# ningyu1991/InclusiveGAN

Measured on AMD Instinct MI355X. Metric: training img/sec (whole node), CelebA 128x128 StyleGAN2+IMLE, higher is better.
Workload: dtype f32-equivalent (3x3 convs: 2-piece fp16 split, operands to <= 1 ulp of fp32, scales per pixel / per channel: no per-tensor window; fp32 sums)

## Files before the change

### include/igan_hip.h

```cpp
#ifndef IGAN_HIP_H
#define IGAN_HIP_H

#include <stddef.h>
#include <stdint.h>

#ifdef __cplusplus
extern "C" {
#endif

#define IGAN_ABI_VERSION 10

typedef void* igan_stream_t;

enum igan_status {
    IGAN_OK = 0,
    IGAN_ERR_INVALID_ARGUMENT = 1,
    IGAN_ERR_HIP = 2,
    IGAN_ERR_UNSUPPORTED = 3
};

int igan_abi_version(void);
size_t igan_struct_size(int which);
const char* igan_last_error(void);

typedef struct igan_upfirdn2d_params {
    const float* x;
    const float* k;
    float* y;
    int upx, upy, downx, downy;
    int padx0, padx1, pady0, pady1;
    int majorDim, inH, inW, minorDim;
    int kernelH, kernelW;
    int outH, outW;
} igan_upfirdn2d_params;

int igan_upfirdn2d(igan_stream_t stream, const igan_upfirdn2d_params* p);
int igan_upfirdn2d_f16(igan_stream_t stream, const igan_upfirdn2d_params* p);
int igan_upfirdn2d_ban(igan_stream_t stream, const igan_upfirdn2d_params* p, const float* noise, const float* strength,
                       int noise_bcast, const float* bias, int act, float alpha, float gain);

typedef struct igan_fused_bias_act_params {
    const float* x;
    const float* b;
    const float* ref;
    float* y;
    int grad;
    int act;
    float alpha;
    float gain;
    int sizeX;
    int sizeB;
    int stepB;
} igan_fused_bias_act_params;

int igan_fused_bias_act(igan_stream_t stream, const igan_fused_bias_act_params* p);
int igan_fused_bias_act_f16(igan_stream_t stream, const igan_fused_bias_act_params* p);

size_t igan_bias_grad_workspace_floats(int sizeX, int sizeB, int stepB);
int igan_bias_grad(igan_stream_t stream, const float* dx, float* db, float* partial,
                   int sizeX, int sizeB, int stepB);

size_t igan_bias_act_noise_workspace_floats(int rows, int C);
int igan_bias_act_noise_fwd(igan_stream_t stream, const float* x, const float* noise, const float* strength,
                            const float* b, float* y, int rows, int C, int act, float alpha, float gain);
int igan_bias_act_noise_bwd(igan_stream_t stream, const float* dy, const float* y, const float* noise,
                            float* dx, float* db, float* dstrength, float* workspace,
                            int rows, int C, int act, float alpha, float gain);

size_t igan_bias_act_noise_dd_workspace_floats(int N, int HW, int C);
int igan_bias_act_noise_bwd_dd(igan_stream_t stream, const float* dy, const float* y, const float* noise, const float* strength,
                               const float* b, const float* dscale, float* dx, float* db, float* dstrength, float* dd,
                               float* workspace, int noise_bcast, int N, int HW, int C, int act, float alpha, float gain);

typedef struct igan_conv2d_params {
    const float* x;
    const float* w;
    float* y;
    const float* in_scale;
    const float* out_scale;
    float* workspace;
    size_t workspace_floats;
    int N, H, W, Cin;
    int OH, OW, Cout;
    int KH, KW;
    int stride, up;
    int pad_y, pad_x;
    int w_transposed;
    int splits;
    int sliced_tiles;
    float alpha;
    const float* bias;
    int act;
    float act_alpha, act_gain;
    const float* noise;
    const float* noise_strength;
    int noise_bcast;
    const void* x_pieces;
    size_t x_pieces_bytes;
    float* x_colmax;
    const void* w_pieces;
    size_t w_pieces_bytes;
} igan_conv2d_params;

int igan_conv2d_plan(const igan_conv2d_params* p, int* splits, int* sliced_tiles, size_t* workspace_floats);
int igan_conv2d(igan_stream_t stream, const igan_conv2d_params* p);
int igan_conv2d_kernel_name(const igan_conv2d_params* p, char* buf, int buflen);

typedef struct igan_conv2d_wgrad_params {
    const float* x;
    const float* dy;
    float* dw;
    const float* in_scale;
    const float* out_scale;
    float* workspace;
    size_t workspace_floats;
    int N, H, W, Cin;
    int OH, OW, Cout;
    int KH, KW;
    int stride, up;
    int pad_y, pad_x;
    int splits;
    float alpha;
    const void* x_pieces;
    const void* dy_pieces;
    size_t x_pieces_bytes;
    size_t dy_pieces_bytes;
    const float* x_colmax;
    const float* dy_colmax;
} igan_conv2d_wgrad_params;

int igan_conv2d_wgrad_plan(const igan_conv2d_wgrad_params* p, int* splits, size_t* workspace_floats);
int igan_conv2d_wgrad(igan_stream_t stream, const igan_conv2d_wgrad_params* p);
int igan_conv2d_wgrad_kernel_name(const igan_conv2d_wgrad_params* p, char* buf, int buflen);

int igan_conv_pieces_wanted(int KH, int KW, int Cin, int Cout);
int igan_pieces_image_ok(int N, int HW, int C);
int igan_conv_piece_form(void);
size_t igan_filter_image_bytes(int KH, int KW, int Cin, int Cout);
int igan_filter_image(igan_stream_t stream, const float* w, void* out, int KH, int KW, int Cin, int Cout, int w_transposed);
size_t igan_colmax_floats(int N, int HW, int C);
int igan_debug_f16_window(unsigned long long* below, unsigned long long* imaged, int reset);
int igan_debug_f16_window_by_kind(unsigned long long* out4, int reset);

int igan_to_pieces(igan_stream_t stream, const float* x, const float* scale, void* out, int N, int HW, int C);

enum { IGAN_DENSE_PRO_NONE = 0, IGAN_DENSE_PRO_SQUARE = 1, IGAN_DENSE_PRO_DEMOD_GRAD = 2 };
enum { IGAN_DENSE_EPI_SCALE = 0, IGAN_DENSE_EPI_BIAS = 1, IGAN_DENSE_EPI_RSQRT = 2, IGAN_DENSE_EPI_STYLE_GRAD = 3 };
typedef struct igan_dense_params {
    const float* x;
    const float* x2;
    const float* w;
    float* y;
    const float* bias;
    const float* e1;
    const float* e2;
    float* colsum;
    int ldx, ldy;
    int M, K, N;
    int w_transposed;
    int prologue, epilogue;
    float alpha, pro_scale, bias_scale, add_const, eps;
} igan_dense_params;
int igan_dense_small(igan_stream_t stream, const igan_dense_params* p);

typedef struct igan_dense_wgrad_params {
    const float* a;
    const float* b;
    const float* b2;
    float* dw;
    int lda;
    int M, K, N;
    int pro_a, pro_b;
    float alpha, pro_scale;
} igan_dense_wgrad_params;
int igan_dense_small_wgrad(igan_stream_t stream, const igan_dense_wgrad_params* p);

#define IGAN_DENSE_MAX_GROUPS 24
#define IGAN_DENSE_MAX_ROWS 64
int igan_dense_small_grouped(igan_stream_t stream, const igan_dense_params* groups, int count);
int igan_dense_small_wgrad_grouped(igan_stream_t stream, const igan_dense_wgrad_params* groups, int count);

int igan_sumsq_taps(igan_stream_t stream, const float* w, float* out, int taps, int n);
int igan_bcast_mul_taps(igan_stream_t stream, const float* w, const float* v, float* out, int taps, int n, float scale);
typedef struct igan_taps_params {
    const float* w;
    const float* v;
    float* out;
    int taps, n;
    float scale;
} igan_taps_params;
int igan_sumsq_taps_grouped(igan_stream_t stream, const igan_taps_params* groups, int count);
int igan_bcast_mul_taps_grouped(igan_stream_t stream, const igan_taps_params* groups, int count);

size_t igan_scale_dot_workspace_floats(int N, int HW, int C);
int igan_scale_dot(igan_stream_t stream, const float* a, const float* b, const float* s, float* out,
                   float* dot, float* workspace, int N, int HW, int C);

int igan_lpips_layer_blocks(int N, int HW);
int igan_lpips_layer_fwd(igan_stream_t stream, const float* fa, const float* fb, const float* lin,
                         float* partial, int N, int HW, int C);
int igan_lpips_layer_bwd(igan_stream_t stream, const float* fa, const float* fb, const float* lin,
                         const float* g, float* dfa, int N, int HW, int C);
int igan_lpips_pairs_fwd(igan_stream_t stream, const float* fa, const float* fb, const float* lin, const int* ia,
                         const int* ib, float* partial, int partial_stride, int blocks, int P, int HW, int C);
int igan_lpips_pairs_bwd(igan_stream_t stream, const float* fa, const float* fb, const float* lin, const int* ia,
                         const int* ib, const float* g, float* dfa, int accumulate, int P, int HW, int C);

int igan_maxpool2x2_fwd(igan_stream_t stream, const float* x, float* y, int N, int H, int W, int C);
int igan_maxpool2x2_bwd(igan_stream_t stream, const float* x, const float* dy, const float* dskip, float* dx,
                        int N, int H, int W, int C);

size_t igan_mbstd_workspace_floats(int N, int H, int W, int C, int G);
int igan_mbstd_fwd(igan_stream_t stream, const float* x, float* y, float* workspace,
                   int N, int H, int W, int C, int G);
int igan_mbstd_bwd(igan_stream_t stream, const float* x, const float* dy, float* dx,
                   int N, int H, int W, int C, int G);

int igan_row_sqnorm(igan_stream_t stream, const float* a, float* out, int rows, int dim);
int igan_nn1_update(igan_stream_t stream, const float* query, const float* qnorm,
                    const float* cand, const float* cnorm, double* best_d2, int* best_idx,
                    float* dots ,
                    int nq, int nc, int dim, int idx_base);

// ... 47 lines not shown
```

### inclusivegan_amd/_abi.py

```python
import ctypes
import os
import threading

_HERE = os.path.dirname(os.path.abspath(__file__))
LIB_PATH = os.environ.get('IGAN_LIB') or os.path.join(_HERE, 'csrc', 'libigan_hip.so')

IGAN_OK = 0
IGAN_ERR_INVALID_ARGUMENT = 1
IGAN_ERR_HIP = 2
IGAN_ERR_UNSUPPORTED = 3

c_float_p = ctypes.POINTER(ctypes.c_float)


class UpFirDn2DParams(ctypes.Structure):
    _fields_ = [
        ('x', ctypes.c_void_p), ('k', ctypes.c_void_p), ('y', ctypes.c_void_p),
        ('upx', ctypes.c_int), ('upy', ctypes.c_int), ('downx', ctypes.c_int), ('downy', ctypes.c_int),
        ('padx0', ctypes.c_int), ('padx1', ctypes.c_int), ('pady0', ctypes.c_int), ('pady1', ctypes.c_int),
        ('majorDim', ctypes.c_int), ('inH', ctypes.c_int), ('inW', ctypes.c_int), ('minorDim', ctypes.c_int),
        ('kernelH', ctypes.c_int), ('kernelW', ctypes.c_int),
        ('outH', ctypes.c_int), ('outW', ctypes.c_int),
    ]


class FusedBiasActParams(ctypes.Structure):
    _fields_ = [
        ('x', ctypes.c_void_p), ('b', ctypes.c_void_p), ('ref', ctypes.c_void_p), ('y', ctypes.c_void_p),
        ('grad', ctypes.c_int), ('act', ctypes.c_int),
        ('alpha', ctypes.c_float), ('gain', ctypes.c_float),
        ('sizeX', ctypes.c_int), ('sizeB', ctypes.c_int), ('stepB', ctypes.c_int),
    ]


class Conv2DParams(ctypes.Structure):
    _fields_ = [
        ('x', ctypes.c_void_p), ('w', ctypes.c_void_p), ('y', ctypes.c_void_p),
        ('in_scale', ctypes.c_void_p), ('out_scale', ctypes.c_void_p),
        ('workspace', ctypes.c_void_p), ('workspace_floats', ctypes.c_size_t),
        ('N', ctypes.c_int), ('H', ctypes.c_int), ('W', ctypes.c_int), ('Cin', ctypes.c_int),
        ('OH', ctypes.c_int), ('OW', ctypes.c_int), ('Cout', ctypes.c_int),
        ('KH', ctypes.c_int), ('KW', ctypes.c_int),
        ('stride', ctypes.c_int), ('up', ctypes.c_int),
        ('pad_y', ctypes.c_int), ('pad_x', ctypes.c_int),
        ('w_transposed', ctypes.c_int), ('splits', ctypes.c_int), ('sliced_tiles', ctypes.c_int), ('alpha', ctypes.c_float),
        ('bias', ctypes.c_void_p), ('act', ctypes.c_int), ('act_alpha', ctypes.c_float), ('act_gain', ctypes.c_float),
        ('noise', ctypes.c_void_p), ('noise_strength', ctypes.c_void_p), ('noise_bcast', ctypes.c_int),
        ('x_pieces', ctypes.c_void_p), ('x_pieces_bytes', ctypes.c_size_t),
        ('x_colmax', ctypes.c_void_p),
        ('w_pieces', ctypes.c_void_p), ('w_pieces_bytes', ctypes.c_size_t),
    ]

    def __init__(self, *args, **kwargs):
        kwargs.setdefault('alpha', 1.0)
        super().__init__(*args, **kwargs)


class Conv2DWgradParams(ctypes.Structure):
    _fields_ = [
        ('x', ctypes.c_void_p), ('dy', ctypes.c_void_p), ('dw', ctypes.c_void_p),
        ('in_scale', ctypes.c_void_p), ('out_scale', ctypes.c_void_p),
        ('workspace', ctypes.c_void_p), ('workspace_floats', ctypes.c_size_t),
        ('N', ctypes.c_int), ('H', ctypes.c_int), ('W', ctypes.c_int), ('Cin', ctypes.c_int),
        ('OH', ctypes.c_int), ('OW', ctypes.c_int), ('Cout', ctypes.c_int),
        ('KH', ctypes.c_int), ('KW', ctypes.c_int),
        ('stride', ctypes.c_int), ('up', ctypes.c_int),
        ('pad_y', ctypes.c_int), ('pad_x', ctypes.c_int),
        ('splits', ctypes.c_int), ('alpha', ctypes.c_float),
        ('x_pieces', ctypes.c_void_p), ('dy_pieces', ctypes.c_void_p), ('x_pieces_bytes', ctypes.c_size_t), ('dy_pieces_bytes', ctypes.c_size_t),
        ('x_colmax', ctypes.c_void_p), ('dy_colmax', ctypes.c_void_p),
    ]

    def __init__(self, *args, **kwargs):
        kwargs.setdefault('alpha', 1.0)
        super().__init__(*args, **kwargs)


class DenseParams(ctypes.Structure):
    _fields_ = [
        ('x', ctypes.c_void_p), ('x2', ctypes.c_void_p), ('w', ctypes.c_void_p), ('y', ctypes.c_void_p),
        ('bias', ctypes.c_void_p), ('e1', ctypes.c_void_p), ('e2', ctypes.c_void_p), ('colsum', ctypes.c_void_p),
        ('ldx', ctypes.c_int), ('ldy', ctypes.c_int),
        ('M', ctypes.c_int), ('K', ctypes.c_int), ('N', ctypes.c_int),
        ('w_transposed', ctypes.c_int),
        ('prologue', ctypes.c_int), ('epilogue', ctypes.c_int),
        ('alpha', ctypes.c_float), ('pro_scale', ctypes.c_float), ('bias_scale', ctypes.c_float),
        ('add_const', ctypes.c_float), ('eps', ctypes.c_float),
    ]


class DenseWgradParams(ctypes.Structure):
    _fields_ = [
        ('a', ctypes.c_void_p), ('b', ctypes.c_void_p), ('b2', ctypes.c_void_p), ('dw', ctypes.c_void_p),
        ('lda', ctypes.c_int),
        ('M', ctypes.c_int), ('K', ctypes.c_int), ('N', ctypes.c_int),
        ('pro_a', ctypes.c_int), ('pro_b', ctypes.c_int),
        ('alpha', ctypes.c_float), ('pro_scale', ctypes.c_float),
    ]


class TapsParams(ctypes.Structure):
    _fields_ = [('w', ctypes.c_void_p), ('v', ctypes.c_void_p), ('out', ctypes.c_void_p),
                ('taps', ctypes.c_int), ('n', ctypes.c_int), ('scale', ctypes.c_float)]


ABI_VERSION = 10
STRUCTS = (UpFirDn2DParams, FusedBiasActParams, Conv2DParams, Conv2DWgradParams, DenseParams, DenseWgradParams, TapsParams)

DENSE_MAX_GROUPS = 24
DENSE_PRO_NONE, DENSE_PRO_SQUARE, DENSE_PRO_DEMOD_GRAD = 0, 1, 2
DENSE_EPI_SCALE, DENSE_EPI_BIAS, DENSE_EPI_RSQRT, DENSE_EPI_STYLE_GRAD = 0, 1, 2, 3

_I, _F, _P, _SZ, _LL = ctypes.c_int, ctypes.c_float, ctypes.c_void_p, ctypes.c_size_t, ctypes.c_longlong

SIGNATURES = {
    'igan_abi_version': (_I, []),
    'igan_struct_size': (_SZ, [_I]),
    'igan_last_error': (ctypes.c_char_p, []),
    'igan_upfirdn2d': (_I, [_P, ctypes.POINTER(UpFirDn2DParams)]),
    'igan_upfirdn2d_f16': (_I, [_P, ctypes.POINTER(UpFirDn2DParams)]),
    'igan_upfirdn2d_ban': (_I, [_P, _P, _P, _P, _I, _P, _I, _F, _F]),
    'igan_fused_bias_act': (_I, [_P, ctypes.POINTER(FusedBiasActParams)]),
    'igan_fused_bias_act_f16': (_I, [_P, ctypes.POINTER(FusedBiasActParams)]),
    'igan_bias_grad_workspace_floats': (_SZ, [_I, _I, _I]),
    'igan_bias_grad': (_I, [_P, _P, _P, _P, _I, _I, _I]),
    'igan_bias_act_noise_workspace_floats': (_SZ, [_I, _I]),
    'igan_bias_act_noise_fwd': (_I, [_P, _P, _P, _P, _P, _P, _I, _I, _I, _F, _F]),
    'igan_bias_act_noise_dd_workspace_floats': (ctypes.c_size_t, [_I, _I, _I]),
    'igan_bias_act_noise_bwd_dd': (_I, [_P, _P, _P, _P, _P, _P, _P, _P, _P, _P, _P, _P, _I, _I, _I, _I, _I, _F, _F]),
    'igan_bias_act_noise_bwd': (_I, [_P, _P, _P, _P, _P, _P, _P, _P, _I, _I, _I, _F, _F]),
    'igan_conv2d_plan': (_I, [ctypes.POINTER(Conv2DParams), ctypes.POINTER(_I), ctypes.POINTER(_I), ctypes.POINTER(_SZ)]),
    'igan_conv2d': (_I, [_P, ctypes.POINTER(Conv2DParams)]),
    'igan_conv2d_kernel_name': (_I, [ctypes.POINTER(Conv2DParams), ctypes.c_char_p, _I]),
    'igan_conv2d_wgrad_kernel_name': (_I, [ctypes.POINTER(Conv2DWgradParams), ctypes.c_char_p, _I]),
    'igan_conv2d_wgrad_plan': (_I, [ctypes.POINTER(Conv2DWgradParams), ctypes.POINTER(_I), ctypes.POINTER(_SZ)]),
    'igan_conv2d_wgrad': (_I, [_P, ctypes.POINTER(Conv2DWgradParams)]),
    'igan_debug_f16_window_by_kind': (_I, [_P, _I]),
    'igan_colmax_floats': (ctypes.c_size_t, [_I, _I, _I]),
    'igan_filter_image_bytes': (ctypes.c_size_t, [_I, _I, _I, _I]),
    'igan_filter_image': (_I, [_P, _P, _P, _I, _I, _I, _I, _I]),
    'igan_to_pieces': (_I, [_P, _P, _P, _P, _I, _I, _I]),
    'igan_conv_pieces_wanted': (_I, [_I, _I, _I, _I]),
    'igan_pieces_image_ok': (_I, [_I, _I, _I]),
    'igan_conv_piece_form': (_I, []),
    'igan_debug_f16_window': (_I, [_P, _P, _I]),
    'igan_dense_small': (_I, [_P, ctypes.POINTER(DenseParams)]),
    'igan_dense_small_wgrad': (_I, [_P, ctypes.POINTER(DenseWgradParams)]),
    'igan_dense_small_grouped': (_I, [_P, ctypes.POINTER(DenseParams), _I]),
    'igan_dense_small_wgrad_grouped': (_I, [_P, ctypes.POINTER(DenseWgradParams), _I]),
    'igan_sumsq_taps_grouped': (_I, [_P, ctypes.POINTER(TapsParams), _I]),
    'igan_bcast_mul_taps_grouped': (_I, [_P, ctypes.POINTER(TapsParams), _I]),
    'igan_sumsq_taps': (_I, [_P, _P, _P, _I, _I]),
    'igan_bcast_mul_taps': (_I, [_P, _P, _P, _P, _I, _I, _F]),
    'igan_scale_dot_workspace_floats': (_SZ, [_I, _I, _I]),
    'igan_scale_dot': (_I, [_P, _P, _P, _P, _P, _P, _P, _I, _I, _I]),
    'igan_lpips_layer_blocks': (_I, [_I, _I]),
    'igan_lpips_layer_fwd': (_I, [_P, _P, _P, _P, _P, _I, _I, _I]),
    'igan_lpips_layer_bwd': (_I, [_P, _P, _P, _P, _P, _P, _I, _I, _I]),
    'igan_lpips_pairs_fwd': (_I, [_P, _P, _P, _P, _P, _P, _P, _I, _I, _I, _I, _I]),
    'igan_lpips_pairs_bwd': (_I, [_P, _P, _P, _P, _P, _P, _P, _P, _I, _I, _I, _I]),
    'igan_maxpool2x2_fwd': (_I, [_P, _P, _P, _I, _I, _I, _I]),
    'igan_maxpool2x2_bwd': (_I, [_P, _P, _P, _P, _P, _I, _I, _I, _I]),
    'igan_mbstd_workspace_floats': (_SZ, [_I, _I, _I, _I, _I]),
    'igan_mbstd_fwd': (_I, [_P, _P, _P, _P, _I, _I, _I, _I, _I]),
    'igan_mbstd_bwd': (_I, [_P, _P, _P, _P, _I, _I, _I, _I, _I]),
    'igan_row_sqnorm': (_I, [_P, _P, _P, _I, _I]),
    'igan_nn1_update': (_I, [_P, _P, _P, _P, _P, _P, _P, _P, _I, _I, _I, _I]),
    'igan_knn_radius_update': (_I, [_P, _P, _P, _P, _P, _P, _P, _I, _I, _I, _I]),
    'igan_manifold_member_update': (_I, [_P, _P, _P, _P, _P, _P, _P, _P, _I, _I, _I, _I]),
    'igan_ppl_endpoints': (_I, [_P, _P, _P, _P, _I, _I, ctypes.c_double, _I]),
    'igan_ppl_crop_prep': (_I, [_P, _P, _P, _I, _I, _I, _I, _I, _I, _I, _I, _I, _LL, _LL, _LL, _LL]),
    'igan_linear_svc_workspace_bytes': (_SZ, [_I, _I, _I]),
    'igan_linear_svc_grad': (_I, [_P, _P, _P, _P, _P, _P, _P, _P, _P, _SZ, _I, _I, _I, ctypes.c_double]),
    'igan_linear_svc_hv': (_I, [_P, _P, _P, _P, _P, _P, _P, _SZ, _I, _I, _I, ctypes.c_double]),
    'igan_linear_svc_linesearch': (_I, [_P, _P, _P, _P, _P, _P, _P, _SZ, _I, _I, _I]),
    'igan_linear_svc_predict': (_I, [_P, _P, _P, _I, _I]),
    'igan_stamp': (_I, [_P, _P]),
    'igan_debug_set_conv_diag': (None, [_P]),
    'igan_stamp_accumulate': (_I, [_P, _P, _P, _I, _I]),
    'igan_finite_check': (_I, [_P, _P, _I, _P]),
    'igan_adam_step': (_I, [_P, _P, _P, _P, _P, _I, _F, _F, _F, _F, _P, _P]),
    'igan_ema': (_I, [_P, _P, _P, _I, _F]),
    'igan_summary_accumulate': (_I, [_P, _P, _I, _P]),
}

_lib = None
_lock = threading.Lock()


class IganError(RuntimeError):
    """HIP-side failure (reference: errors::Internal -> tf.errors.InternalError)."""


def get_plugin():
    global _lib
    if _lib is not None:
        return _lib
    with _lock:
        if _lib is not None:
            return _lib
        if not os.path.isfile(LIB_PATH):
            raise ImportError(
                'inclusivegan_amd: %s is missing. Build it with `python -c "import __graft_entry__ as g; g.build()"` '
                'or `make -C inclusivegan_amd/csrc`. There is no CPU fallback.' % LIB_PATH)
        import torch
        lib = ctypes.CDLL(LIB_PATH)
        for name, (restype, argtypes) in SIGNATURES.items():
            fn = getattr(lib, name)
            fn.restype = restype
            fn.argtypes = argtypes
        if lib.igan_abi_version() != ABI_VERSION:
            raise ImportError('inclusivegan_amd: libigan_hip.so has ABI version %d, this binding needs %d -- rebuild it '
                              '(make -C inclusivegan_amd/csrc)' % (lib.igan_abi_version(), ABI_VERSION))
        for which, struct in enumerate(STRUCTS):
            if lib.igan_struct_size(which) != ctypes.sizeof(struct):
                raise ImportError('inclusivegan_amd: libigan_hip.so was built with sizeof(%s) = %d, this binding declares %d -- '
                                  'rebuild it' % (struct.__name__, lib.igan_struct_size(which), ctypes.sizeof(struct)))
        _lib = lib
    return _lib


# ... 10 lines not shown
```

### inclusivegan_amd/csrc/bias_act_noise.hip

```cpp
#include "igan_common.h"

namespace {

struct BanArgs {
    const float* x;
    const float* ref;
    const float* noise;
    const float* strength;
    const float* b;
    float* y;
    float* partial;
    int rows, C;
    int act;
    float alpha, gain;
};

__device__ __forceinline__ float act_fwd(int act, float v, float alpha) {
    if (act == 2) return v > 0.f ? v : 0.f;
    if (act == 3) return v > 0.f ? v : v * alpha;
    return v;
}
__device__ __forceinline__ float act_bwd(int act, float dy, float y, float alpha) {
    if (act == 2) return y > 0.f ? dy : 0.f;
    if (act == 3) return y > 0.f ? dy : dy * alpha;
    return dy;
}

__global__ __launch_bounds__(256) void ban_fwd_kernel(BanArgs a) {
    const int cv = a.C >> 2;
    const long long n4 = (long long)a.rows * cv;
    const float s = (a.noise && a.strength) ? *a.strength : 0.f;
    const float4* x4 = reinterpret_cast<const float4*>(a.x);
    float4* y4 = reinterpret_cast<float4*>(a.y);
    for (long long i = (long long)blockIdx.x * blockDim.x + threadIdx.x; i < n4; i += (long long)gridDim.x * blockDim.x) {
        const int row = (int)(i / cv);
        const int c = (int)(i - (long long)row * cv) << 2;
        float4 v = x4[i];
        float add = a.noise ? a.noise[row] * s : 0.f;
        float4 bb = a.b ? *reinterpret_cast<const float4*>(a.b + c) : make_float4(0.f, 0.f, 0.f, 0.f);
        v.x = act_fwd(a.act, v.x + add + bb.x, a.alpha) * a.gain;
        v.y = act_fwd(a.act, v.y + add + bb.y, a.alpha) * a.gain;
        v.z = act_fwd(a.act, v.z + add + bb.z, a.alpha) * a.gain;
        v.w = act_fwd(a.act, v.w + add + bb.w, a.alpha) * a.gain;
        y4[i] = v;
    }
}

__global__ __launch_bounds__(256) void ban_bwd_kernel(BanArgs a) {
    __shared__ float4 red[256];
    __shared__ float reds[256];
    const int cv = a.C >> 2;
    const int cvt = min(cv, 256);
    const int rl = 256 / cvt;
    const int col = threadIdx.x % cvt + blockIdx.y * 256;
    const int lane_r = threadIdx.x / cvt;
    const bool active = (col < cv) && (lane_r < rl);
    const int rows_per_block = (a.rows + gridDim.x - 1) / gridDim.x;
    const int r0 = blockIdx.x * rows_per_block;
    const int r1 = min(r0 + rows_per_block, a.rows);
    const float4* dy4 = reinterpret_cast<const float4*>(a.x);
    const float4* y4 = reinterpret_cast<const float4*>(a.ref);
    float4* dx4 = reinterpret_cast<float4*>(a.y);
    float4 accb = make_float4(0.f, 0.f, 0.f, 0.f);
    float accs = 0.f;
    if (active) {
        for (int rb = r0 + lane_r; rb < r1; rb += 4 * rl) {
            float4 g[4], yy[4];
            float nz[4];
#pragma unroll
            for (int u = 0; u < 4; u++) {
                const int r = min(rb + u * rl, r1 - 1);
                const long long i = (long long)r * cv + col;
                g[u] = dy4[i];
                yy[u] = y4[i];
                nz[u] = a.noise ? a.noise[r] : 0.f;
            }
#pragma unroll
            for (int u = 0; u < 4; u++) {
                const int r = rb + u * rl;
                if (r < r1) {
                    float4 d;
                    d.x = act_bwd(a.act, g[u].x, yy[u].x, a.alpha) * a.gain;
                    d.y = act_bwd(a.act, g[u].y, yy[u].y, a.alpha) * a.gain;
                    d.z = act_bwd(a.act, g[u].z, yy[u].z, a.alpha) * a.gain;
                    d.w = act_bwd(a.act, g[u].w, yy[u].w, a.alpha) * a.gain;
                    dx4[(long long)r * cv + col] = d;
                    accb.x += d.x; accb.y += d.y; accb.z += d.z; accb.w += d.w;
                    accs += nz[u] * ((d.x + d.y) + (d.z + d.w));
                }
            }
        }
    }
    red[threadIdx.x] = accb;
    reds[threadIdx.x] = accs;
    __syncthreads();
    if (threadIdx.x < cvt && col < cv) {
        float4 t = red[threadIdx.x];
        for (int j = 1; j < rl; j++) {
            const float4 u = red[threadIdx.x + j * cvt];
            t.x += u.x; t.y += u.y; t.z += u.z; t.w += u.w;
        }
        float* p = a.partial + (size_t)blockIdx.x * (a.C + 1) + (size_t)col * 4;
        p[0] = t.x; p[1] = t.y; p[2] = t.z; p[3] = t.w;
    }
    if (a.noise && blockIdx.y == 0) {
        float s = reds[threadIdx.x];
#pragma unroll
        for (int off = 32; off > 0; off >>= 1) s += __shfl_down(s, off, 64);
        __syncthreads();
        if ((threadIdx.x & 63) == 0) reds[threadIdx.x >> 6] = s;
        __syncthreads();
        if (threadIdx.x == 0) a.partial[(size_t)blockIdx.x * (a.C + 1) + a.C] = (reds[0] + reds[1]) + (reds[2] + reds[3]);
    } else if (!a.noise && blockIdx.y == 0 && threadIdx.x == 0) {
        a.partial[(size_t)blockIdx.x * (a.C + 1) + a.C] = 0.f;
    }
}

__global__ __launch_bounds__(256) void ban_final_kernel(const float* partial, float* db, float* dstrength, int blocks, int C) {
    __shared__ float red[256];
    const int c = blockIdx.x * 16 + (threadIdx.x & 15);
    const int grp = threadIdx.x >> 4;
    float s = 0.f;
    if (c <= C) {
        float s0 = 0.f, s1 = 0.f, s2 = 0.f, s3 = 0.f;
        int j = grp;
        for (; j + 48 < blocks; j += 64) {
            s0 += partial[(size_t)j * (C + 1) + c];        s1 += partial[(size_t)(j + 16) * (C + 1) + c];
            s2 += partial[(size_t)(j + 32) * (C + 1) + c]; s3 += partial[(size_t)(j + 48) * (C + 1) + c];
        }
        for (; j < blocks; j += 16) s0 += partial[(size_t)j * (C + 1) + c];
        s = (s0 + s1) + (s2 + s3);
    }
    red[threadIdx.x] = s;
    __syncthreads();
    if (grp == 0 && c <= C) {
        float t = 0.f;
#pragma unroll
        for (int g = 0; g < 16; g++) t += red[g * 16 + threadIdx.x];
        if (c < C) { if (db) db[c] = t; }
        else if (dstrength) *dstrength = t;
    }
}

__global__ __launch_bounds__(256) void ban_bwd_dd_kernel(BanArgs a, const float* __restrict__ strength_p, int HW, int bps) {
    __shared__ float4 red[256];
    __shared__ float4 red2[256];
    __shared__ float reds[256];
    const int cv = a.C >> 2;
    const int cvt = min(cv, 256);
    const int rl = 256 / cvt;
    const int col = threadIdx.x % cvt + blockIdx.y * 256;
    const int lane_r = threadIdx.x / cvt;
    const bool active = (col < cv) && (lane_r < rl);
    const int n = blockIdx.x / bps, j = blockIdx.x - n * bps;
    const int per = (HW + bps - 1) / bps;
    const int r0 = n * HW + j * per;
    const int r1 = min(r0 + per, (n + 1) * HW);
    const float4* dy4 = reinterpret_cast<const float4*>(a.x);
    const float4* y4 = reinterpret_cast<const float4*>(a.ref);
    float4* dx4 = reinterpret_cast<float4*>(a.y);
    const float st = (a.noise && strength_p) ? strength_p[0] : 0.f;
    const float inv_gain = 1.0f / a.gain;
    const float inv_neg = (a.act == 3) ? 1.0f / (a.gain * a.alpha) : inv_gain;
    float4 bb = make_float4(0.f, 0.f, 0.f, 0.f);
    if (active && a.b) bb = *reinterpret_cast<const float4*>(a.b + 4 * col);
    float4 accb = make_float4(0.f, 0.f, 0.f, 0.f), accd = make_float4(0.f, 0.f, 0.f, 0.f);
    float accs = 0.f;
    if (active) {
        for (int rb = r0 + lane_r; rb < r1; rb += 4 * rl) {
            float4 g[4], yy[4];
            float nz[4];
#pragma unroll
            for (int u = 0; u < 4; u++) {
                const int r = min(rb + u * rl, r1 - 1);
                const long long i = (long long)r * cv + col;
                g[u] = dy4[i];
                yy[u] = y4[i];
                nz[u] = a.noise ? a.noise[a.rows < 0 ? r - n * HW : r] : 0.f;
            }
#pragma unroll
            for (int u = 0; u < 4; u++) {
                const int r = rb + u * rl;
                if (r < r1) {
                    float4 d;
                    d.x = act_bwd(a.act, g[u].x, yy[u].x, a.alpha) * a.gain;
                    d.y = act_bwd(a.act, g[u].y, yy[u].y, a.alpha) * a.gain;
                    d.z = act_bwd(a.act, g[u].z, yy[u].z, a.alpha) * a.gain;
                    d.w = act_bwd(a.act, g[u].w, yy[u].w, a.alpha) * a.gain;
                    dx4[(long long)r * cv + col] = d;
                    accb.x += d.x; accb.y += d.y; accb.z += d.z; accb.w += d.w;
                    accs += nz[u] * ((d.x + d.y) + (d.z + d.w));
                    const float off = nz[u] * st;
                    accd.x += d.x * (yy[u].x * (yy[u].x >= 0.f ? inv_gain : inv_neg) - bb.x - off);
                    accd.y += d.y * (yy[u].y * (yy[u].y >= 0.f ? inv_gain : inv_neg) - bb.y - off);
                    accd.z += d.z * (yy[u].z * (yy[u].z >= 0.f ? inv_gain : inv_neg) - bb.z - off);
                    accd.w += d.w * (yy[u].w * (yy[u].w >= 0.f ? inv_gain : inv_neg) - bb.w - off);
                }
            }
        }
    }
    red[threadIdx.x] = accb;
    red2[threadIdx.x] = accd;
    reds[threadIdx.x] = accs;
    __syncthreads();
    const int W = 2 * a.C + 1;
    if (threadIdx.x < cvt && col < cv) {
        float4 t = red[threadIdx.x], t2 = red2[threadIdx.x];
        for (int k = 1; k < rl; k++) {
            const float4 u = red[threadIdx.x + k * cvt], u2 = red2[threadIdx.x + k * cvt];
            t.x += u.x; t.y += u.y; t.z += u.z; t.w += u.w;
            t2.x += u2.x; t2.y += u2.y; t2.z += u2.z; t2.w += u2.w;
        }
        float* p = a.partial + (size_t)blockIdx.x * W + (size_t)col * 4;
        p[0] = t.x; p[1] = t.y; p[2] = t.z; p[3] = t.w;
        float* q = p + a.C + 1;
        q[0] = t2.x; q[1] = t2.y; q[2] = t2.z; q[3] = t2.w;
    }
    if (blockIdx.y == 0) {
        float s = a.noise ? reds[threadIdx.x] : 0.f;
#pragma unroll
        for (int off = 32; off > 0; off >>= 1) s += __shfl_down(s, off, 64);
        __syncthreads();
        if ((threadIdx.x & 63) == 0) reds[threadIdx.x >> 6] = s;
        __syncthreads();
        if (threadIdx.x == 0) a.partial[(size_t)blockIdx.x * W + a.C] = (reds[0] + reds[1]) + (reds[2] + reds[3]);
    }
}

__global__ __launch_bounds__(256) void ban_dd_final_kernel(const float* partial, const float* dscale, float* db, float* dstrength, float* dd,
                                                           int N, int bps, int C) {
    __shared__ float red[256];
    const int W = 2 * C + 1;
    const int c = blockIdx.x * 16 + (threadIdx.x & 15);
    const int grp = threadIdx.x >> 4;
    const bool sample = blockIdx.y > 0;
    const int n = (int)blockIdx.y - 1;
    const int b0 = sample ? n * bps : 0, b1 = sample ? (n + 1) * bps : N * bps;
    const int off = sample ? C + 1 : 0;
    const int cmax = sample ? C - 1 : C;
    float s = 0.f;
    if (c <= cmax) {
        float s0 = 0.f, s1 = 0.f, s2 = 0.f, s3 = 0.f;
        int j = b0 + grp;
        for (; j + 48 < b1; j += 64) {
            s0 += partial[(size_t)j * W + off + c];        s1 += partial[(size_t)(j + 16) * W + off + c];
            s2 += partial[(size_t)(j + 32) * W + off + c]; s3 += partial[(size_t)(j + 48) * W + off + c];
        }
        for (; j < b1; j += 16) s0 += partial[(size_t)j * W + off + c];
        s = (s0 + s1) + (s2 + s3);
    }
    red[threadIdx.x] = s;
    __syncthreads();
    if (grp == 0 && c <= cmax) {
        float t = 0.f;
#pragma unroll
        for (int g = 0; g < 16; g++) t += red[g * 16 + threadIdx.x];
        if (sample) { if (dd) dd[(size_t)n * C + c] = t / dscale[(size_t)n * C + c]; }
        else if (c < C) { if (db) db[c] = t; }
        else if (dstrength) *dstrength = t;
    }
}

int ban_dd_bps(int N, int HW, int C) {
    const int cvt = std::min(C / 4, 256);
    const int rl = 256 / cvt;
    return std::max(1, std::min(std::max(512 / std::max(N, 1), 1), std::max(HW / (rl * 8), 1)));
}

int ban_blocks(int rows, int C) {
    const int cvt = std::min(C / 4, 256);
    const int rl = 256 / cvt;
    int b = rows / (rl * 8);
    return std::max(1, std::min(b, 512));
}

int ban_check(const char* who, int rows, int C, int act, float gain) {
    IGAN_REQUIRE(gain > 0.0f, "%s: gain must be positive (the derivative is keyed on the sign of y)", who);
    IGAN_REQUIRE(rows >= 1 && C >= 4 && (C % 4) == 0, "%s: needs channel-minor data with C %% 4 == 0", who);
    IGAN_REQUIRE((long long)rows * C <= INT32_MAX, "%s: x is too large", who);
    IGAN_REQUIRE(act >= 1 && act <= 3, "%s: only linear / relu / lrelu (act 1..3) are offered here", who);
    return IGAN_OK;
}

}

extern "C" size_t igan_bias_act_noise_workspace_floats(int rows, int C) {
    if (rows <= 0 || C < 4) return 0;
    return (size_t)ban_blocks(rows, C) * (size_t)(C + 1);
}

extern "C" size_t igan_bias_act_noise_dd_workspace_floats(int N, int HW, int C) {
    if (N <= 0 || HW <= 0 || C < 4) return 0;
    return (size_t)N * ban_dd_bps(N, HW, C) * (size_t)(2 * C + 1);
}

extern "C" int igan_bias_act_noise_bwd_dd(igan_stream_t stream_, const float* dy, const float* y, const float* noise, const float* strength,
                                          const float* b, const float* dscale, float* dx, float* db, float* dstrength, float* dd,
                                          float* workspace, int noise_bcast, int N, int HW, int C, int act, float alpha, float gain) {
    using namespace igan;
    IGAN_REQUIRE(dy && y && dx && workspace && dscale && dd, "bias_act_noise_bwd_dd: null buffer");
    IGAN_REQUIRE((noise == nullptr) || (strength != nullptr && dstrength != nullptr), "bias_act_noise_bwd_dd: noise given without strength / dstrength");
    IGAN_REQUIRE(N >= 1 && HW >= 1 && (long long)N * HW <= INT32_MAX, "bias_act_noise_bwd_dd: bad sizes");
    if (int rc = ban_check("bias_act_noise_bwd_dd", N * HW, C, act, gain)) return rc;
    IGAN_REQUIRE(noise == nullptr || C <= 1024, "bias_act_noise_bwd_dd: with noise C must be <= 1024 (the noise-strength partial is reduced by the first block column only)");
    IGAN_REQUIRE(act == 1 || act == 3, "bias_act_noise_bwd_dd: the pre-activation value is recovered from y: linear or lrelu only");
    IGAN_REQUIRE(act != 3 || alpha > 0.0f, "bias_act_noise_bwd_dd: lrelu slope must be positive");
    IGAN_REQUIRE((((uintptr_t)dy | (uintptr_t)y | (uintptr_t)dx | (uintptr_t)b) & 15) == 0, "bias_act_noise_bwd_dd: buffers must be 16-byte aligned");
    BanArgs a{dy, y, noise, nullptr, b, dx, workspace, noise_bcast ? -1 : N * HW, C, act, alpha, gain};
    const int bps = ban_dd_bps(N, HW, C);
    dim3 grid(N * bps, ceil_div(C / 4, 256));
    hipLaunchKernelGGL(ban_bwd_dd_kernel, grid, dim3(256), 0, (hipStream_t)stream_, a, strength, HW, bps);
    hipLaunchKernelGGL(ban_dd_final_kernel, dim3(ceil_div(C + 1, 16), 1 + N), dim3(256), 0, (hipStream_t)stream_,
                       (const float*)workspace, dscale, db, noise ? dstrength : nullptr, dd, N, bps, C);
    IGAN_LAUNCH_CHECK("bias_act_noise_bwd_dd launch");
    return IGAN_OK;
}

extern "C" int igan_bias_act_noise_fwd(igan_stream_t stream_, const float* x, const float* noise, const float* strength,
                                       const float* b, float* y, int rows, int C, int act, float alpha, float gain) {
    using namespace igan;
    IGAN_REQUIRE(x && y, "bias_act_noise_fwd: null buffer");
    IGAN_REQUIRE((noise == nullptr) == (strength == nullptr), "bias_act_noise_fwd: noise and strength go together");
    if (int rc = ban_check("bias_act_noise_fwd", rows, C, act, gain)) return rc;
    IGAN_REQUIRE((((uintptr_t)x | (uintptr_t)y | (uintptr_t)b) & 15) == 0, "bias_act_noise_fwd: buffers must be 16-byte aligned");
    BanArgs a{x, nullptr, noise, strength, b, y, nullptr, rows, C, act, alpha, gain};
    const long long n4 = (long long)rows * (C / 4);
    const int grid = (int)std::min<long long>(ceil_div_ll(n4, 256), 256 * 16);
    hipLaunchKernelGGL(ban_fwd_kernel, dim3(grid), dim3(256), 0, (hipStream_t)stream_, a);
    IGAN_LAUNCH_CHECK("bias_act_noise_fwd launch");
    return IGAN_OK;
}

extern "C" int igan_bias_act_noise_bwd(igan_stream_t stream_, const float* dy, const float* y, const float* noise,
                                       float* dx, float* db, float* dstrength, float* workspace,
                                       int rows, int C, int act, float alpha, float gain) {
    using namespace igan;
    IGAN_REQUIRE(dy && y && dx && workspace, "bias_act_noise_bwd: null buffer");
    IGAN_REQUIRE((noise == nullptr) || (dstrength != nullptr), "bias_act_noise_bwd: noise given without dstrength");
    if (int rc = ban_check("bias_act_noise_bwd", rows, C, act, gain)) return rc;
    IGAN_REQUIRE((((uintptr_t)dy | (uintptr_t)y | (uintptr_t)dx) & 15) == 0, "bias_act_noise_bwd: buffers must be 16-byte aligned");
    BanArgs a{dy, y, noise, nullptr, nullptr, dx, workspace, rows, C, act, alpha, gain};
    const int blocks = ban_blocks(rows, C);
    dim3 grid(blocks, ceil_div(C / 4, 256));
    hipLaunchKernelGGL(ban_bwd_kernel, grid, dim3(256), 0, (hipStream_t)stream_, a);
    hipLaunchKernelGGL(ban_final_kernel, dim3(ceil_div(C + 1, 16)), dim3(256), 0, (hipStream_t)stream_,
                       (const float*)workspace, db, noise ? dstrength : nullptr, blocks, C);
    IGAN_LAUNCH_CHECK("bias_act_noise_bwd launch");
    return IGAN_OK;
}
```

### inclusivegan_amd/csrc/conv2d_mfma.hip

```cpp
#include "igan_common.h"
#include <cmath>
#include <cstdlib>
#include <type_traits>

namespace {

typedef float f32x16 __attribute__((ext_vector_type(16)));

constexpr int BK = 32;
#ifndef IGAN_SPLIT
#define IGAN_SPLIT 8
#endif
constexpr int LDK = BK + 4;

struct ConvArgs {
    const float* x;
    const float* w;
    float* y;
    float* out;
    const float* in_scale;
    const float* out_scale;
    int N, H, W, Cin;
    int OH, OW, Cout;
    int KH, KW;
    int stride, up_shift;
    int pad_y, pad_x;
    int splits;
    int full_tiles;
    int nx, ny;
    int cpt;
    int Mtot;
    int vecA, vecB, vecS;
    int vecY;
    float alpha;
    int xcd_remap;
    int b_scale;
    int prio;
    int walk;
    int stagger;
    unsigned long long* diag;
    const float* bias;
    int act;
    float act_alpha, act_gain;
    const float* noise;
    const float* noise_strength;
    int noise_bcast;
    int diag_mode;
    const unsigned short* xp;
    const unsigned short* wp;
};

__device__ __forceinline__ float noise_term(const ConvArgs& a, int pix) {
    if (a.noise == nullptr || pix < 0) return 0.0f;
    return a.noise[a.noise_bcast ? pix % (a.OH * a.OW) : pix] * a.noise_strength[0];
}

__device__ __forceinline__ float epi_act(int act, float v, float alpha) {
    if (act == 2) return v > 0.f ? v : 0.f;
    if (act == 3) return v > 0.f ? v : v * alpha;
    return v;
}

__device__ __forceinline__ float4 f4zero() { return make_float4(0.f, 0.f, 0.f, 0.f); }
__device__ __forceinline__ float4 f4mul(float4 a, float4 b) { return make_float4(a.x * b.x, a.y * b.y, a.z * b.z, a.w * b.w); }
__device__ __forceinline__ float4 f4sel(bool has, float4 s) { return make_float4(has ? s.x : 1.f, has ? s.y : 1.f, has ? s.z : 1.f, has ? s.w : 1.f); }

typedef unsigned int u32x4 __attribute__((ext_vector_type(4)));
constexpr unsigned OOB = 0x7FFFFFF0u;

__device__ __forceinline__ __amdgpu_buffer_rsrc_t make_rsrc(const float* p, unsigned bytes) {
    return __builtin_amdgcn_make_buffer_rsrc(const_cast<float*>(p), 0, (int)bytes, 0x00020000);
}

struct LoadAddr {
    unsigned off;
    int left;
};
template <bool VEC>
__device__ __forceinline__ LoadAddr make_addr(int off, int left) {
    LoadAddr a;
    if constexpr (VEC) { a.off = (left > 0) ? (unsigned)off * 4u : OOB; a.left = 0; }
    else { a.off = (unsigned)off * 4u; a.left = left; }
    return a;
// ... 833 lines not shown
        o[q] = __builtin_bit_cast(unsigned short, b);
        r -= (float)b;
    }
}

__global__ __launch_bounds__(256) void to_planes_kernel(const float* __restrict__ x, const float* __restrict__ scale, unsigned short* __restrict__ out,
                                                         int total, int cpp, int C, int HW) {
    const int idx = min((int)(blockIdx.x * 256 + threadIdx.x), total - 1);
    const int p = idx / cpp, c = idx - p * cpp;
    const float4* src = reinterpret_cast<const float4*>(x + (size_t)p * C + 16 * c);
    float v[16];
#pragma unroll
    for (int i = 0; i < 4; i++) { const float4 f = src[i]; v[4 * i] = f.x; v[4 * i + 1] = f.y; v[4 * i + 2] = f.z; v[4 * i + 3] = f.w; }
    if (scale != nullptr) {
        const float4* sc = reinterpret_cast<const float4*>(scale + (size_t)(p / HW) * C + 16 * c);
#pragma unroll
        for (int i = 0; i < 4; i++) { const float4 f = sc[i]; v[4 * i] *= f.x; v[4 * i + 1] *= f.y; v[4 * i + 2] *= f.z; v[4 * i + 3] *= f.w; }
    }
    unsigned short pc[3][16];
#pragma unroll
    for (int i = 0; i < 16; i++) {
        unsigned short o[3];
        split3(v[i], o);
        pc[0][i] = o[0]; pc[1][i] = o[1]; pc[2][i] = o[2];
    }
    __shared__ uint4 stage[256 * 6];
#pragma unroll
    for (int q = 0; q < 3; q++)
#pragma unroll
        for (int hh = 0; hh < 2; hh++) {
            uint4 u;
            u.x = pc[q][8 * hh + 0] | ((unsigned)pc[q][8 * hh + 1] << 16); u.y = pc[q][8 * hh + 2] | ((unsigned)pc[q][8 * hh + 3] << 16);
            u.z = pc[q][8 * hh + 4] | ((unsigned)pc[q][8 * hh + 5] << 16); u.w = pc[q][8 * hh + 6] | ((unsigned)pc[q][8 * hh + 7] << 16);
            stage[threadIdx.x * 6 + 2 * q + hh] = u;
        }
    __syncthreads();
    const int units = min(256, total - (int)blockIdx.x * 256);
    uint4* dst = reinterpret_cast<uint4*>(out + (size_t)blockIdx.x * 256 * 48);
#pragma unroll
    for (int k = 0; k < 6; k++) {
        const int j = k * 256 + threadIdx.x;
        if (j < units * 6) dst[j] = stage[j];
    }
}

template <bool WT>
__global__ __launch_bounds__(256) void filter_planes_kernel(const float* __restrict__ w, unsigned short* __restrict__ out, int taps, int KW_, int Nn, int K) {
    const int cpk = K >> 4;
    const int idx = blockIdx.x * 256 + threadIdx.x;
    if (idx >= taps * Nn * cpk) return;
    int tap, n, c;
    if constexpr (WT) { c = idx % cpk; const int r = idx / cpk; n = r % Nn; tap = r / Nn; }
    else { n = idx % Nn; const int r = idx / Nn; c = r % cpk; tap = r / cpk; }
    float v[16];
    if constexpr (WT) {
        const float4* src = reinterpret_cast<const float4*>(w + ((size_t)(taps - 1 - tap) * Nn + n) * K + 16 * c);
#pragma unroll
        for (int i = 0; i < 4; i++) { const float4 f = src[i]; v[4 * i] = f.x; v[4 * i + 1] = f.y; v[4 * i + 2] = f.z; v[4 * i + 3] = f.w; }
    } else {
#pragma unroll
        for (int i = 0; i < 16; i++) v[i] = w[((size_t)tap * K + 16 * c + i) * Nn + n];
    }
    unsigned short pc[3][16];
#pragma unroll
    for (int i = 0; i < 16; i++) {
        unsigned short o[3];
        split3(v[i], o);
        pc[0][i] = o[0]; pc[1][i] = o[1]; pc[2][i] = o[2];
    }
    uint4* dst = reinterpret_cast<uint4*>(out + (((size_t)c * taps + tap) * Nn + n) * 48);
#pragma unroll
    for (int q = 0; q < 3; q++)
#pragma unroll
        for (int hh = 0; hh < 2; hh++) {
            uint4 u;
            u.x = pc[q][8 * hh + 0] | ((unsigned)pc[q][8 * hh + 1] << 16); u.y = pc[q][8 * hh + 2] | ((unsigned)pc[q][8 * hh + 3] << 16);
            u.z = pc[q][8 * hh + 4] | ((unsigned)pc[q][8 * hh + 5] << 16); u.w = pc[q][8 * hh + 6] | ((unsigned)pc[q][8 * hh + 7] << 16);
            dst[2 * q + hh] = u;
        }
}


typedef _Float16 f16x8 __attribute__((ext_vector_type(8)));
constexpr int H_COLBLOCKS = 1024;
constexpr int H_KSK = 2;
__device__ unsigned long long g_f16_below_window = 0ull, g_f16_imaged = 0ull;
__device__ unsigned long long g_f16_below_window_cols = 0ull, g_f16_imaged_cols = 0ull;

__host__ __device__ inline size_t align256(size_t b) { return (b + 255) & ~(size_t)255; }
inline size_t rows_part_bytes(size_t P_, size_t C) { return align256(4 * P_ * C + 4 * P_); }
inline size_t cols_part_bytes(size_t P_, size_t C) { return align256(4 * P_ * C + 8 * C + 4 * (size_t)H_COLBLOCKS * C); }
inline size_t filter_part_bytes(size_t taps, size_t Nn, size_t K) { return align256(4 * taps * Nn * K + 4 * Nn + 4 * taps * H_KSK * Nn); }

__device__ __forceinline__ float scale_from_amax(float amax) {
    int e = (int)((__float_as_uint(amax) >> 23) & 0xFFu);
    e = max(15, min(e, 254));
    return __uint_as_float((unsigned)(268 - e) << 23);
}
__device__ __forceinline__ float inv_scale_from_amax(float amax) {
    int e = (int)((__float_as_uint(amax) >> 23) & 0xFFu);
    e = max(15, min(e, 254));
    return __uint_as_float((unsigned)(e - 14) << 23);
}
__device__ __forceinline__ void count_window(int below, unsigned long long* counter) {
#ifdef IGAN_NO_WINDOW_COUNT
    return;
#endif
#pragma unroll
    for (int o = 32; o >= 1; o >>= 1) below += __shfl_xor(below, o);
    if ((threadIdx.x & 63) == 0 && below != 0) atomicAdd(counter, (unsigned long long)below);
}

__device__ __forceinline__ void split2(float vs, unsigned short (&o)[2]) {
    const _Float16 p0 = (_Float16)vs;
    const _Float16 p1 = (_Float16)((vs - (float)p0) * 2048.0f);
    o[0] = __builtin_bit_cast(unsigned short, p0);
    o[1] = __builtin_bit_cast(unsigned short, p1);
}

__device__ __forceinline__ void load_unit16(const float* __restrict__ x, const float* __restrict__ scale, int p, int c, int C, int HW, float (&v)[16]) {
    const float4* src = reinterpret_cast<const float4*>(x + (size_t)p * C + 16 * c);
#pragma unroll
    for (int i = 0; i < 4; i++) { const float4 f = src[i]; v[4 * i] = f.x; v[4 * i + 1] = f.y; v[4 * i + 2] = f.z; v[4 * i + 3] = f.w; }
    if (scale != nullptr) {
        const float4* sc = reinterpret_cast<const float4*>(scale + (size_t)(p / HW) * C + 16 * c);
#pragma unroll
        for (int i = 0; i < 4; i++) { const float4 f = sc[i]; v[4 * i] *= f.x; v[4 * i + 1] *= f.y; v[4 * i + 2] *= f.z; v[4 * i + 3] *= f.w; }
    }
}
__device__ __forceinline__ void store_units(const unsigned short (&pc)[2][16], uint4* stage, unsigned short* __restrict__ out, int total, int chunk) {
#pragma unroll
    for (int q = 0; q < 2; q++)
#pragma unroll
        for (int hh = 0; hh < 2; hh++) {
            uint4 u;
            u.x = pc[q][8 * hh + 0] | ((unsigned)pc[q][8 * hh + 1] << 16); u.y = pc[q][8 * hh + 2] | ((unsigned)pc[q][8 * hh + 3] << 16);
            u.z = pc[q][8 * hh + 4] | ((unsigned)pc[q][8 * hh + 5] << 16); u.w = pc[q][8 * hh + 6] | ((unsigned)pc[q][8 * hh + 7] << 16);
            stage[threadIdx.x * 4 + 2 * q + hh] = u;
        }
    __syncthreads();
    const int units = min(256, total - chunk * 256);
    uint4* dst = reinterpret_cast<uint4*>(out + (size_t)chunk * 256 * 32);
#pragma unroll
    for (int k = 0; k < 4; k++) {
        const int j = k * 256 + threadIdx.x;
        if (j < units * 4) dst[j] = stage[j];
    }
}

__global__ __launch_bounds__(256) void rows_f16_kernel(const float* __restrict__ x, const float* __restrict__ scale, unsigned short* __restrict__ out,
                                                        float* __restrict__ rowinv, float* __restrict__ colmax, int total, int cpp, int lcpp, int C, int HW) {
    __shared__ uint4 stage[256 * 4];
    const int c = threadIdx.x & (cpp - 1);
    float cm[16];
#pragma unroll
    for (int i = 0; i < 16; i++) cm[i] = 0.0f;
    int below = 0;
    const int nchunks = (total + 255) >> 8;
    for (int chunk = blockIdx.x; chunk < nchunks; chunk += gridDim.x) {
        const bool mine = chunk * 256 + (int)threadIdx.x < total;
        const int idx = min(chunk * 256 + (int)threadIdx.x, total - 1);
        const int p = idx >> lcpp;
        float v[16];
        load_unit16(x, scale, p, c, C, HW, v);
        float m = 0.0f;
#pragma unroll
        for (int i = 0; i < 16; i++) { const float av = fabsf(v[i]); m = fmaxf(m, av); if (mine) cm[i] = fmaxf(cm[i], av); }
        for (int o = 1; o < cpp; o <<= 1) m = fmaxf(m, __shfl_xor(m, o));
        const float S = scale_from_amax(m);
        if (mine && c == 0) rowinv[p] = inv_scale_from_amax(m);
        unsigned short pc[2][16];
#pragma unroll
        for (int i = 0; i < 16; i++) {
            unsigned short o[2];
            const float vs = v[i] * S;
            split2(vs, o);
            pc[0][i] = o[0]; pc[1][i] = o[1];
            below += (mine && vs != 0.0f && fabsf(vs) < 0x1p-12f) ? 1 : 0;
        }
        if (chunk != (int)blockIdx.x) __syncthreads();
        store_units(pc, stage, out, total, chunk);
    }
    count_window(below, &g_f16_below_window);
#ifndef IGAN_NO_WINDOW_COUNT
    if (blockIdx.x == 0 && threadIdx.x == 0) atomicAdd(&g_f16_imaged, (unsigned long long)total * 16ull);
#endif
    if (colmax != nullptr) {
        __syncthreads();
        float* sm = reinterpret_cast<float*>(stage);
#pragma unroll
        for (int i = 0; i < 16; i++) sm[threadIdx.x * 16 + i] = cm[i];
        __syncthreads();
        const int groups = 256 >> lcpp;
        for (int ch = threadIdx.x; ch < C; ch += 256) {
            const int cc = ch >> 4, i = ch & 15;
            float m = 0.0f;
            for (int j = 0; j < groups; j++) m = fmaxf(m, sm[(j * cpp + cc) * 16 + i]);
            colmax[4 + (size_t)blockIdx.x * C + ch] = m;
        }
        if (blockIdx.x == 0 && threadIdx.x == 0) colmax[0] = (float)gridDim.x;
    }
}

__global__ __launch_bounds__(256) void cols_amax_kernel(const float* __restrict__ x, const float* __restrict__ scale, float* __restrict__ partial,
                                                         int P_, int C4, int lC4, int HW, float* __restrict__ header) {
    if (header != nullptr && blockIdx.x == 0 && threadIdx.x == 0) header[0] = (float)gridDim.x;
    __shared__ float4 red[256];
    const int q = threadIdx.x & (C4 - 1), pl = threadIdx.x >> lC4, ppi = 256 >> lC4;
    const int step = gridDim.x * ppi;
    float4 m = make_float4(0.f, 0.f, 0.f, 0.f);
    auto take = [&](int p) {
        float4 v = reinterpret_cast<const float4*>(x)[(size_t)p * C4 + q];
        if (scale != nullptr) {
            const float4 f = reinterpret_cast<const float4*>(scale)[(size_t)(p / HW) * C4 + q];
            v.x *= f.x; v.y *= f.y; v.z *= f.z; v.w *= f.w;
        }
        m.x = fmaxf(m.x, fabsf(v.x)); m.y = fmaxf(m.y, fabsf(v.y)); m.z = fmaxf(m.z, fabsf(v.z)); m.w = fmaxf(m.w, fabsf(v.w));
    };
    int p = blockIdx.x * ppi + pl;
    for (; p + step < P_; p += 2 * step) { take(p); take(p + step); }
    if (p < P_) take(p);
    red[threadIdx.x] = m;
    __syncthreads();
    if (pl == 0) {
        for (int j = 1; j < ppi; j++) {
            const float4 o = red[j * C4 + q];
            m.x = fmaxf(m.x, o.x); m.y = fmaxf(m.y, o.y); m.z = fmaxf(m.z, o.z); m.w = fmaxf(m.w, o.w);
        }
        reinterpret_cast<float4*>(partial)[(size_t)blockIdx.x * C4 + q] = m;
    }
}
__global__ __launch_bounds__(256) void cols_finalize_kernel(const float* __restrict__ partial, float* __restrict__ inv, float* __restrict__ sc, int rows, int C, const float* __restrict__ header) {
    __shared__ float red[256];
    if (header != nullptr) rows = (int)header[0];
    const int c = blockIdx.x * 8 + (threadIdx.x & 7), rl = threadIdx.x >> 3;
    float m0 = 0.0f, m1 = 0.0f, m2 = 0.0f, m3 = 0.0f;
    if (c < C) {
        int r = rl;
        for (; r + 96 < rows; r += 128) {
            m0 = fmaxf(m0, partial[(size_t)r * C + c]); m1 = fmaxf(m1, partial[(size_t)(r + 32) * C + c]);
            m2 = fmaxf(m2, partial[(size_t)(r + 64) * C + c]); m3 = fmaxf(m3, partial[(size_t)(r + 96) * C + c]);
        }
        for (; r < rows; r += 32) m0 = fmaxf(m0, partial[(size_t)r * C + c]);
    }
    red[threadIdx.x] = fmaxf(fmaxf(m0, m1), fmaxf(m2, m3));
    __syncthreads();
    if (rl == 0 && c < C) {
        float m = red[threadIdx.x];
        for (int j = 1; j < 32; j++) m = fmaxf(m, red[8 * j + threadIdx.x]);
        inv[c] = inv_scale_from_amax(m);
        sc[c] = scale_from_amax(m);
    }
}
__global__ __launch_bounds__(256) void cols_f16_kernel(const float* __restrict__ x, const float* __restrict__ scale, unsigned short* __restrict__ out,
                                                        const float* __restrict__ sc, int total, int cpp, int C, int HW) {
    __shared__ uint4 stage[256 * 4];
    const bool mine = (int)(blockIdx.x * 256 + threadIdx.x) < total;
    const int idx = min((int)(blockIdx.x * 256 + threadIdx.x), total - 1);
    const int p = idx / cpp, c = idx - p * cpp;
    float v[16], S[16];
    load_unit16(x, scale, p, c, C, HW, v);
#pragma unroll
    for (int i = 0; i < 4; i++) { const float4 f = reinterpret_cast<const float4*>(sc + 16 * c)[i]; S[4 * i] = f.x; S[4 * i + 1] = f.y; S[4 * i + 2] = f.z; S[4 * i + 3] = f.w; }
    unsigned short pc[2][16];
    int below = 0;
#pragma unroll
    for (int i = 0; i < 16; i++) {
        unsigned short o[2];
        const float vs = v[i] * S[i];
        split2(vs, o);
        pc[0][i] = o[0]; pc[1][i] = o[1];
        below += (mine && vs != 0.0f && fabsf(vs) < 0x1p-12f) ? 1 : 0;
    }
    count_window(below, &g_f16_below_window_cols);
#ifndef IGAN_NO_WINDOW_COUNT
    if (blockIdx.x == 0 && threadIdx.x == 0) atomicAdd(&g_f16_imaged_cols, (unsigned long long)total * 16ull);
#endif
    store_units(pc, stage, out, total, (int)blockIdx.x);
}

template <bool WT>
__global__ __launch_bounds__(256) void filter_amax_kernel(const float* __restrict__ w, float* __restrict__ partial, int taps, int Nn, int K) {
    if constexpr (WT) {
        const int row = blockIdx.x * 4 + (threadIdx.x >> 6), lane = threadIdx.x & 63;
        if (row >= taps * Nn) return;
        const float4* src = reinterpret_cast<const float4*>(w + (size_t)row * K);
        float m = 0.0f;
        for (int i = lane; i < (K >> 2); i += 64) { const float4 f = src[i]; m = fmaxf(m, fmaxf(fmaxf(fabsf(f.x), fabsf(f.y)), fmaxf(fabsf(f.z), fabsf(f.w)))); }
#pragma unroll
        for (int o = 32; o >= 1; o >>= 1) m = fmaxf(m, __shfl_xor(m, o));
        if (lane == 0) partial[row] = m;
    } else {
        __shared__ float red[256];
        const int tap = blockIdx.x / H_KSK, j = blockIdx.x - tap * H_KSK;
        const int n = blockIdx.y * 64 + (threadIdx.x & 63), rl = threadIdx.x >> 6;
        const int k0 = (int)(((long long)j * K) / H_KSK), k1 = (int)(((long long)(j + 1) * K) / H_KSK);
        float m = 0.0f;
        if (n < Nn) {
            const float* src = w + (size_t)tap * K * Nn + n;
            int k = k0 + rl;
            for (; k + 28 < k1; k += 32) {
                float v[8];
#pragma unroll
                for (int i = 0; i < 8; i++) v[i] = fabsf(src[(size_t)(k + 4 * i) * Nn]);
                m = fmaxf(m, fmaxf(fmaxf(fmaxf(v[0], v[1]), fmaxf(v[2], v[3])), fmaxf(fmaxf(v[4], v[5]), fmaxf(v[6], v[7]))));
            }
            for (; k < k1; k += 4) m = fmaxf(m, fabsf(src[(size_t)k * Nn]));
        }
        red[threadIdx.x] = m;
        __syncthreads();
        if (rl == 0 && n < Nn) partial[(size_t)blockIdx.x * Nn + n] = fmaxf(fmaxf(m, red[64 + threadIdx.x]), fmaxf(red[128 + threadIdx.x], red[192 + threadIdx.x]));
    }
}

template <bool WT>
__global__ __launch_bounds__(256) void filter_planes_f16_kernel(const float* __restrict__ w, unsigned short* __restrict__ out, float* __restrict__ inv,
                                                                 const float* __restrict__ partial, int prow, int taps, int KW_, int Nn, int K) {
    const int cpk = K >> 4;
    const int idx = blockIdx.x * 256 + threadIdx.x;
    if (idx >= taps * Nn * cpk) return;
    int tap, n, c;
    if constexpr (WT) { c = idx % cpk; const int r = idx / cpk; n = r % Nn; tap = r / Nn; }
    else { n = idx % Nn; const int r = idx / Nn; c = r % cpk; tap = r / cpk; }
    float amax = 0.0f;
    {
        float m0 = 0.f, m1 = 0.f, m2 = 0.f, m3 = 0.f, m4 = 0.f, m5 = 0.f;
        int r = 0;
        for (; r + 6 <= prow; r += 6) {
            const float* q = partial + (size_t)r * Nn + n;
            const float v0 = q[0], v1 = q[Nn], v2 = q[2 * (size_t)Nn], v3 = q[3 * (size_t)Nn], v4 = q[4 * (size_t)Nn], v5 = q[5 * (size_t)Nn];
            m0 = fmaxf(m0, v0); m1 = fmaxf(m1, v1); m2 = fmaxf(m2, v2); m3 = fmaxf(m3, v3); m4 = fmaxf(m4, v4); m5 = fmaxf(m5, v5);
        }
        for (; r < prow; r++) m0 = fmaxf(m0, partial[(size_t)r * Nn + n]);
        amax = fmaxf(fmaxf(fmaxf(m0, m1), fmaxf(m2, m3)), fmaxf(m4, m5));
    }
    const float S = scale_from_amax(amax);
    if (tap == 0 && c == 0) inv[n] = inv_scale_from_amax(amax);
    float v[16];
    if constexpr (WT) {
        const float4* src = reinterpret_cast<const float4*>(w + ((size_t)(taps - 1 - tap) * Nn + n) * K + 16 * c);
#pragma unroll
        for (int i = 0; i < 4; i++) { const float4 f = src[i]; v[4 * i] = f.x; v[4 * i + 1] = f.y; v[4 * i + 2] = f.z; v[4 * i + 3] = f.w; }
    } else {
#pragma unroll
        for (int i = 0; i < 16; i++) v[i] = w[((size_t)tap * K + 16 * c + i) * Nn + n];
    }
    unsigned short pc[2][16];
#pragma unroll
    for (int i = 0; i < 16; i++) {
        unsigned short o[2];
        split2(v[i] * S, o);
        pc[0][i] = o[0]; pc[1][i] = o[1];
    }
    uint4* dst = reinterpret_cast<uint4*>(out + (((size_t)c * taps + tap) * Nn + n) * 32);
#pragma unroll
// ... 1386 lines not shown
    if (a.in_scale) hipLaunchKernelGGL((conv_fwd_kernel<BM, BN, WM, WN, WT, VEC, true>), grid, dim3(WM * WN * 64), 0, stream, a);
    else hipLaunchKernelGGL((conv_fwd_kernel<BM, BN, WM, WN, WT, VEC, false>), grid, dim3(WM * WN * 64), 0, stream, a);
}

template <int BM, int BN, int WM, int WN>
void launch_fwd(hipStream_t stream, const ConvArgs& a, dim3 grid, bool wt, bool vec) {
    if (wt) {
        if (vec) launch_fwd2<BM, BN, WM, WN, true, true>(stream, a, grid);
        else launch_fwd2<BM, BN, WM, WN, true, false>(stream, a, grid);
    } else {
        if (vec) launch_fwd2<BM, BN, WM, WN, false, true>(stream, a, grid);
        else launch_fwd2<BM, BN, WM, WN, false, false>(stream, a, grid);
    }
}

}

namespace {

int device_cus() {
    static int cus = 0;
    if (cus == 0) {
        int n = 256, dev = 0;
        hipDeviceProp_t prop;
        if (hipGetDevice(&dev) == hipSuccess && hipGetDeviceProperties(&prop, dev) == hipSuccess && prop.multiProcessorCount > 0)
            n = prop.multiProcessorCount;
        (void)hipGetLastError();
        cus = n;
    }
    return cus;
}

struct TileList { int nx, ny, T, rem; };
TileList tile_list(const igan_conv2d_params* p, const FwdTile& t, int Mmax, int nclass) {
    TileList l;
    l.nx = igan::ceil_div(Mmax, t.BM);
    l.ny = igan::ceil_div(p->Cout, t.BN);
    l.T = l.nx * l.ny * nclass;
    l.rem = l.T % device_cus();
    return l;
}


bool use_dma_kernel(const igan_conv2d_params* p, const FwdTile& t, bool walk) {
    static const bool dma = !(getenv("IGAN_CONV_DMA") && atoi(getenv("IGAN_CONV_DMA")) == 0);
    if (!dma || t.BM != 128 || t.BN != 128 || !walk || !eight_waves("IGAN_CONV_8WAVE")) return false;
    if ((long long)p->N * p->OH * p->OW >= (1LL << 24)) return false;
    if (p->in_scale) {
        const int up = p->up;
        for (int c = 0; c < up * up; c++) {
            const int qh = (p->OH - c / up + up - 1) / up, qw = (p->OW - c % up + up - 1) / up;
            if (qh <= 0 || qw <= 0) continue;
            const int samples = 127 / (qh * qw) + 2;
            if ((long long)std::min(samples, p->N) * p->Cin > 2048) return false;
        }
    }
    return true;
}

bool walk_ok(const igan_conv2d_params* p) {
    static const bool walk = !(getenv("IGAN_CONV_WALK") && atoi(getenv("IGAN_CONV_WALK")) == 0);
    const bool wt = p->w_transposed != 0;
    const bool vecA = (p->Cin % 4 == 0) && (((uintptr_t)p->x & 15) == 0);
    const bool vecS = (p->Cin % 4 == 0) && (((uintptr_t)p->in_scale & 15) == 0);
    const bool vecB = ((wt ? p->Cin : p->Cout) % 4 == 0) && (((uintptr_t)p->w & 15) == 0);
    return walk && vecA && vecB && (p->in_scale == nullptr || vecS) && (p->Cin % BK == 0);
}

int planes_mode() {
    static const int mode = [] { const char* v = getenv("IGAN_CONV_PLANES"); const int m = v ? atoi(v) : 2; return m == 0 ? 0 : (m == 1 ? 1 : 2); }();
    return mode;
}
bool planes_enabled() { return planes_mode() != 0; }

int ilog2(int v) { int l = 0; while ((1 << l) < v) ++l; return l; }
bool pow2(int v) { return v > 0 && (v & (v - 1)) == 0; }

void launch_piece_image(hipStream_t stream, const float* x, const float* scale, unsigned short* out, int P_, int HW, int C) {
    const int cpp = C / PK, total = P_ * cpp;
    hipLaunchKernelGGL(to_planes_kernel, dim3(igan::ceil_div(total, 256)), dim3(256), 0, stream, x, scale, out, total, cpp, C, HW);
}
void launch_row_image(hipStream_t stream, const float* x, const float* scale, unsigned short* out, int P_, int HW, int C, float* colmax) {
    const int cpp = C / PK, total = P_ * cpp;
    float* rowinv = reinterpret_cast<float*>(reinterpret_cast<unsigned char*>(out) + (size_t)P_ * C * 4);
    const int nchunks = igan::ceil_div(total, 256);
    const int grid = colmax ? std::min(nchunks, H_COLBLOCKS) : nchunks;
    hipLaunchKernelGGL(rows_f16_kernel, dim3(grid), dim3(256), 0, stream, x, scale, out, rowinv, colmax, total, cpp, ilog2(cpp), C, HW);
}
void launch_colmax_only(hipStream_t stream, const float* x, const float* scale, float* colmax, int P_, int HW, int C) {
    const int C4 = C / 4, ppi = 256 / C4;
    const int blocks = std::min(H_COLBLOCKS, igan::ceil_div(P_, ppi));
    hipLaunchKernelGGL(cols_amax_kernel, dim3(blocks), dim3(256), 0, stream, x, scale, colmax + 4, P_, C4, ilog2(C4), HW, colmax);
}
void launch_col_image(hipStream_t stream, const float* x, const float* scale, unsigned short* out, int P_, int HW, int C, const float* colmax) {
    const int cpp = C / PK, total = P_ * cpp, C4 = C / 4;
    float* inv = reinterpret_cast<float*>(reinterpret_cast<unsigned char*>(out) + (size_t)P_ * C * 4);
    float* sc = inv + C;
    float* partial = sc + C;
    const int ppi = 256 / C4;
    const int blocks = std::min(H_COLBLOCKS, igan::ceil_div(P_, ppi));
    if (colmax == nullptr) {
        hipLaunchKernelGGL(cols_amax_kernel, dim3(blocks), dim3(256), 0, stream, x, scale, partial, P_, C4, ilog2(C4), HW, (float*)nullptr);
        hipLaunchKernelGGL(cols_finalize_kernel, dim3(igan::ceil_div(C, 8)), dim3(256), 0, stream, (const float*)partial, inv, sc, blocks, C, (const float*)nullptr);
    } else
        hipLaunchKernelGGL(cols_finalize_kernel, dim3(igan::ceil_div(C, 8)), dim3(256), 0, stream, colmax + 4, inv, sc, 0, C, colmax);
    hipLaunchKernelGGL(cols_f16_kernel, dim3(igan::ceil_div(total, 256)), dim3(256), 0, stream, x, scale, out, (const float*)sc, total, cpp, C, HW);
}
bool f16_tap_outer() { static const int v = getenv("IGAN_F16_TAP_OUTER") ? atoi(getenv("IGAN_F16_TAP_OUTER")) : 1; return v != 0; }
bool f16_w4() { static const int v = getenv("IGAN_F16_W4") ? atoi(getenv("IGAN_F16_W4")) : 1; return v != 0; }
void launch_filter_image(hipStream_t stream, const float* w, unsigned short* wp, bool wt, int taps, int KW_, int Nn, int K) {
    const int wtotal = taps * Nn * (K / PK);
    if (planes_mode() == 2) {
        float* inv = reinterpret_cast<float*>(reinterpret_cast<unsigned char*>(wp) + (size_t)taps * Nn * K * 4);
        float* partial = inv + Nn;
        if (wt) {
            hipLaunchKernelGGL((filter_amax_kernel<true>), dim3(igan::ceil_div(taps * Nn, 4)), dim3(256), 0, stream, w, partial, taps, Nn, K);
            hipLaunchKernelGGL((filter_planes_f16_kernel<true>), dim3(igan::ceil_div(wtotal, 256)), dim3(256), 0, stream, w, wp, inv, (const float*)partial, taps, taps, KW_, Nn, K);
        } else {
            hipLaunchKernelGGL((filter_amax_kernel<false>), dim3(taps * H_KSK, igan::ceil_div(Nn, 64)), dim3(256), 0, stream, w, partial, taps, Nn, K);
            hipLaunchKernelGGL((filter_planes_f16_kernel<false>), dim3(igan::ceil_div(wtotal, 256)), dim3(256), 0, stream, w, wp, inv, (const float*)partial, taps * H_KSK, taps, KW_, Nn, K);
        }
    } else {
        if (wt) hipLaunchKernelGGL((filter_planes_kernel<true>), dim3(igan::ceil_div(wtotal, 256)), dim3(256), 0, stream, w, wp, taps, KW_, Nn, K);
        else hipLaunchKernelGGL((filter_planes_kernel<false>), dim3(igan::ceil_div(wtotal, 256)), dim3(256), 0, stream, w, wp, taps, KW_, Nn, K);
    }
}

bool planes_shape_ok(const igan_conv2d_params* p, const FwdTile& t, int Mmax) {
    if (!planes_enabled() || t.BM != 128 || t.BN != 128 || p->Cin % BK != 0) return false;
    static const int min_rows = getenv("IGAN_PLANES_MIN_ROWS") ? atoi(getenv("IGAN_PLANES_MIN_ROWS")) : 1024;
    if (p->KH * p->KW == 1 || (long long)p->KH * p->KW * p->Cin < 1152 || Mmax < min_rows) return false;
    if ((long long)p->N * p->OH * p->OW >= (1LL << 24)) return false;
    if ((long long)p->N * p->H * p->W * p->Cin * 6 >= 0x7FFFFF00LL || (long long)p->KH * p->KW * p->Cin * p->Cout * 6 >= 0x7FFFFF00LL) return false;
    if (planes_mode() == 2 && (!pow2(p->Cin / PK) || p->Cin / PK > 64 || p->KH * p->KW > 9 || p->Cout % 4 != 0)) return false;
#ifdef IGAN_DIAGNOSTIC
    {
        static const int only_cin = getenv("IGAN_PLANES_ONLY_CIN") ? atoi(getenv("IGAN_PLANES_ONLY_CIN")) : 0;
        static const int no_act = getenv("IGAN_PLANES_NO_ACT") ? atoi(getenv("IGAN_PLANES_NO_ACT")) : 0;
        static const int no_scale = getenv("IGAN_PLANES_NO_SCALE") ? atoi(getenv("IGAN_PLANES_NO_SCALE")) : 0;
        static const int kind = getenv("IGAN_PLANES_KIND") ? atoi(getenv("IGAN_PLANES_KIND")) : 0;
        static const int wt = getenv("IGAN_PLANES_WT") ? atoi(getenv("IGAN_PLANES_WT")) : 0;
        if (only_cin && p->Cin != only_cin) return false;
        if ((no_act == 1 && p->act != 0) || (no_act == 2 && p->act == 0)) return false;
        if ((no_scale == 1 && p->in_scale != nullptr) || (no_scale == 2 && p->in_scale == nullptr)) return false;
        if ((kind == 1 && (p->stride != 1 || p->up != 1)) || (kind == 2 && p->stride != 2) || (kind == 3 && p->up != 2)) return false;
        if ((wt == 1 && p->w_transposed) || (wt == 2 && !p->w_transposed)) return false;
    }
#endif
    return true;
}
bool use_planes_kernel(const igan_conv2d_params* p, const FwdTile& t, int Mmax) {
    if (!planes_shape_ok(p, t, Mmax) || (((uintptr_t)p->x | (uintptr_t)p->w | (uintptr_t)p->in_scale | (uintptr_t)p->x_pieces) & 15) != 0) return false;
    if (planes_mode() == 2 && (((uintptr_t)p->y | (uintptr_t)p->out_scale | (uintptr_t)p->bias) & 15) != 0) return false;
    return true;
}
size_t planes_x_floats(const igan_conv2d_params* p) {
    if (planes_mode() == 2) return rows_part_bytes((size_t)p->N * p->H * p->W, (size_t)p->Cin) / 4;
    return (size_t)p->N * p->H * p->W * p->Cin * 6 / 4;
}
size_t planes_w_floats(const igan_conv2d_params* p) {
    if (planes_mode() == 2) return filter_part_bytes((size_t)p->KH * p->KW, (size_t)p->Cout, (size_t)p->Cin) / 4;
    return (size_t)p->KH * p->KW * p->Cin * p->Cout * 6 / 4;
}

}

static unsigned long long* g_conv_diag = nullptr;
// ... 104 lines not shown
    if (is_small_dense(p)) {
        colmax_own_pass();
        IGAN_REQUIRE(p->noise == nullptr, "conv2d: the fused noise epilogue is not offered on the small dense path");
        dense_small(stream, p->x, p->w, p->y, p->N, p->Cin, p->Cout, p->w_transposed != 0, p->alpha);
        IGAN_LAUNCH_CHECK("conv2d dense launch");
        return IGAN_OK;
    }
    if (const int kind = thin_conv_kind(p)) {
        colmax_own_pass();
        IGAN_REQUIRE(p->noise == nullptr, "conv2d: the fused noise epilogue is not offered on the thin-channel path");
        thin_conv(stream, p, kind);
        IGAN_LAUNCH_CHECK("conv2d thin-channel launch");
        return IGAN_OK;
    }
    int Mmax, chunks_max, nclass;
    fwd_counts(p, Mmax, chunks_max, nclass);
    const FwdTile t = pick_fwd_tile(Mmax, p->Cout);
    const TileList l = tile_list(p, t, Mmax, nclass);
    int splits = std::max(1, p->splits);
    const int sliced = std::min(std::max(p->sliced_tiles, 0), l.T);
    if (sliced == 0) splits = 1;
    const size_t partial_floats = (splits > 1) ? (size_t)sliced * splits * t.BM * t.BN : 0;
    const bool planes = use_planes_kernel(p, t, Mmax) && p->workspace != nullptr &&
                        p->workspace_floats >= partial_floats + planes_x_floats(p) + planes_w_floats(p);
    if (splits > 1) {
        IGAN_REQUIRE(p->workspace != nullptr, "conv2d: splits > 1 needs a workspace");
        IGAN_REQUIRE(p->workspace_floats >= partial_floats, "conv2d: workspace too small");
    }
    if (splits > 1 || planes) IGAN_REQUIRE((((uintptr_t)p->workspace) & 15) == 0, "conv2d: workspace must be 16-byte aligned");

    ConvArgs a;
    a.x = p->x; a.w = p->w;
    a.y = (splits > 1) ? p->workspace : nullptr;
    a.out = p->y;
    a.in_scale = p->in_scale; a.out_scale = p->out_scale;
    a.N = p->N; a.H = p->H; a.W = p->W; a.Cin = p->Cin;
    a.OH = p->OH; a.OW = p->OW; a.Cout = p->Cout;
    a.KH = p->KH; a.KW = p->KW;
    a.stride = p->stride; a.up_shift = (p->up == 2) ? 1 : 0;
    a.pad_y = p->pad_y; a.pad_x = p->pad_x;
    a.splits = splits;
    a.nx = l.nx; a.ny = l.ny;
    a.full_tiles = (splits > 1) ? l.T - sliced : l.T;
    a.cpt = ceil_div(p->Cin, BK);
    a.Mtot = p->N * p->OH * p->OW;
    a.vecA = (p->Cin % 4 == 0) && (((uintptr_t)p->x & 15) == 0);
    a.vecS = (p->Cin % 4 == 0) && (((uintptr_t)p->in_scale & 15) == 0);
    if (p->w_transposed) a.vecB = (p->Cin % 4 == 0) && (((uintptr_t)p->w & 15) == 0);
    else a.vecB = (p->Cout % 4 == 0) && (((uintptr_t)p->w & 15) == 0);
    a.vecY = (p->Cout % 2 == 0) && ((((uintptr_t)p->y | (uintptr_t)p->out_scale) & 7) == 0);
    a.alpha = p->alpha;
    {
        static const bool remap = !(getenv("IGAN_XCD_REMAP") && atoi(getenv("IGAN_XCD_REMAP")) == 0);
        a.xcd_remap = remap ? 1 : 0;
        static const bool walk = !(getenv("IGAN_CONV_WALK") && atoi(getenv("IGAN_CONV_WALK")) == 0);
        a.diag = g_conv_diag;
        static const int stagger = getenv("IGAN_CONV_STAGGER") ? atoi(getenv("IGAN_CONV_STAGGER")) : 0;
        a.stagger = stagger;
        static const bool bscale = !(getenv("IGAN_CONV_BSCALE") && atoi(getenv("IGAN_CONV_BSCALE")) == 0);
        a.b_scale = bscale ? 1 : 0;
        static const bool pprio = !(getenv("IGAN_CONV_PROLOGUE_PRIO") && atoi(getenv("IGAN_CONV_PROLOGUE_PRIO")) == 0);
        a.prio = pprio ? 1 : 0;
        a.walk = (walk && a.vecA && a.vecB && (a.in_scale == nullptr || a.vecS) && (p->Cin % BK == 0)) ? 1 : 0;
    }
    a.bias = p->bias; a.act = p->act; a.act_alpha = p->act_alpha; a.act_gain = p->act_gain;
    a.noise = p->act ? p->noise : nullptr; a.noise_strength = p->noise_strength; a.noise_bcast = p->noise_bcast;
    a.xp = nullptr; a.wp = nullptr;
    a.diag_mode = 0;
#ifdef IGAN_DIAGNOSTIC
    a.diag_mode = getenv("IGAN_DIAG_MODE") ? atoi(getenv("IGAN_DIAG_MODE")) : 0;
#endif

    dim3 grid(a.full_tiles + (l.T - a.full_tiles) * splits);
    const bool wt = p->w_transposed != 0;
    const bool vec = a.vecA && a.vecB && (a.in_scale == nullptr || a.vecS);
    bool launched = false;
    if (!planes) colmax_own_pass();
    if (planes) {
        IGAN_REQUIRE(p->x_pieces == nullptr || planes_mode() == 1, "conv2d: the two-piece fp16 form writes its own images (one scale per pixel here, per channel in the weight gradient): x_pieces must be NULL");
        IGAN_REQUIRE(p->x_pieces == nullptr || p->x_pieces_bytes == planes_x_floats(p) * 4, "conv2d: x_pieces is not the image of this x (x_pieces_bytes != N*H*W*Cin*6)");
        const unsigned short* xp = reinterpret_cast<const unsigned short*>(p->x_pieces);
        unsigned short* wp = reinterpret_cast<unsigned short*>(p->workspace + partial_floats + planes_x_floats(p));
        const int cpp = p->Cin / PK;
        if (xp == nullptr) {
            unsigned short* own = reinterpret_cast<unsigned short*>(p->workspace + partial_floats);
            if (a.diag_mode & 1) {}
            else if (planes_mode() == 2) launch_row_image(stream, p->x, p->in_scale, own, p->N * p->H * p->W, p->H * p->W, p->Cin, p->x_colmax);
            else launch_piece_image(stream, p->x, p->in_scale, own, p->N * p->H * p->W, p->H * p->W, p->Cin);
            xp = own;
        }
        if (p->w_pieces != nullptr) {
            IGAN_REQUIRE(p->w_pieces_bytes == igan_filter_image_bytes(p->KH, p->KW, p->Cin, p->Cout) && (((uintptr_t)p->w_pieces) & 15) == 0,
                         "conv2d: w_pieces is not an image igan_filter_image() wrote for this filter (size / alignment)");
            wp = reinterpret_cast<unsigned short*>(const_cast<void*>(p->w_pieces));
        } else if (!(a.diag_mode & 1)) launch_filter_image(stream, p->w, wp, wt, p->KH * p->KW, p->KW, p->Cout, p->Cin);
        a.xp = xp; a.wp = wp;
        a.cpt = cpp;
        if (a.diag_mode & 2) {}
        else if (planes_mode() == 2) {
            const bool tapo = f16_tap_outer();
            if (tapo && f16_w4()) hipLaunchKernelGGL(conv_fwd_planes_w4_kernel, grid, dim3(256), 0, stream, a);
            else if (tapo) hipLaunchKernelGGL((conv_fwd_planes_kernel<2, true>), grid, dim3(512), 0, stream, a);
            else hipLaunchKernelGGL((conv_fwd_planes_kernel<2, false>), grid, dim3(512), 0, stream, a);
        } else hipLaunchKernelGGL((conv_fwd_planes_kernel<3>), grid, dim3(512), 0, stream, a);
        IGAN_LAUNCH_CHECK("conv2d (piece form) launch");
        launched = true;
    } else
    if (use_dma_kernel(p, t, a.walk != 0)) {
        if (wt) {
            if (a.in_scale) hipLaunchKernelGGL((conv_fwd_dma_kernel<true, true>), grid, dim3(512), 0, stream, a);
            else hipLaunchKernelGGL((conv_fwd_dma_kernel<true, false>), grid, dim3(512), 0, stream, a);
        } else {
            if (a.in_scale) hipLaunchKernelGGL((conv_fwd_dma_kernel<false, true>), grid, dim3(512), 0, stream, a);
            else hipLaunchKernelGGL((conv_fwd_dma_kernel<false, false>), grid, dim3(512), 0, stream, a);
        }
        IGAN_LAUNCH_CHECK("conv2d (LDS-DMA) launch");
        launched = true;
    }
    if (launched) {}
    else if (t.BM == 128 && t.BN == 128 && eight_waves("IGAN_CONV_8WAVE")) launch_fwd<128, 128, 2, 4>(stream, a, grid, wt, vec);
    else if (t.BM == 128 && t.BN == 128) launch_fwd<128, 128, 2, 2>(stream, a, grid, wt, vec);
    else if (t.BM == 128 && t.BN == 64 && eight_waves("IGAN_CONV_8WAVE")) launch_fwd<128, 64, 4, 2>(stream, a, grid, wt, vec);
    else if (t.BM == 128 && t.BN == 64) launch_fwd<128, 64, 2, 2>(stream, a, grid, wt, vec);
    else if (t.BM == 128 && t.BN == 32) launch_fwd<128, 32, 4, 1>(stream, a, grid, wt, vec);
    else launch_fwd<32, 128, 1, 4>(stream, a, grid, wt, vec);
    IGAN_LAUNCH_CHECK("conv2d launch");

    if (splits > 1) {
        const int rp = std::max(2, std::min(t.BM, t.BM / ceil_div(1024, sliced)));
        hipLaunchKernelGGL(conv_fixup_kernel, dim3(sliced, ceil_div(t.BM, rp)), dim3(256), 0, stream, a, t.BM, t.BN, rp);
        IGAN_LAUNCH_CHECK("conv2d fix-up launch");
    }
    return IGAN_OK;
}

namespace {

int wgrad_geometry_check(const igan_conv2d_wgrad_params* p) {
    IGAN_REQUIRE(p->x && p->dy && p->dw, "conv2d_wgrad: null buffer");
    IGAN_REQUIRE(p->N >= 1 && p->H >= 1 && p->W >= 1 && p->Cin >= 1, "conv2d_wgrad: input dims must be positive");
    IGAN_REQUIRE(p->OH >= 1 && p->OW >= 1 && p->Cout >= 1, "conv2d_wgrad: output dims must be positive");
    IGAN_REQUIRE(p->KH >= 1 && p->KW >= 1, "conv2d_wgrad: kernel must be at least 1x1");
    IGAN_REQUIRE(p->stride >= 1 && p->up >= 1, "conv2d_wgrad: stride and up must be at least 1");
    IGAN_REQUIRE(p->stride == 1 || p->up == 1, "conv2d_wgrad: at most one of stride, up may exceed 1");
    if (!(p->up == 1 || p->up == 2)) return igan::fail(IGAN_ERR_UNSUPPORTED, "conv2d_wgrad: up must be 1 or 2 (got %d)", p->up);
    IGAN_REQUIRE((long long)p->N * p->H * p->W * p->Cin * 4 <= 0x7FFFFFF0LL, "conv2d_wgrad: input too large (2 GiB per operand)");
    IGAN_REQUIRE((long long)p->N * p->OH * p->OW * p->Cout * 4 <= 0x7FFFFFF0LL, "conv2d_wgrad: output gradient too large (2 GiB per operand)");
    IGAN_REQUIRE((long long)p->KH * p->KW * p->Cin * p->Cout <= INT32_MAX, "conv2d_wgrad: filter too large");
    return IGAN_OK;
}

template <int BM, int BN, int WM, int WN, bool VEC>
void launch_wgrad2(hipStream_t stream, const WgradArgs& a, dim3 grid, int scm) {
    if constexpr (BM == 128 && BN == 128 && WM * WN == 8) {
        hipLaunchKernelGGL((conv_wgrad_kernel<BM, BN, WM, WN, VEC, 0>), grid, dim3(WM * WN * 64), 0, stream, a);
    } else {
        if (scm == 0) hipLaunchKernelGGL((conv_wgrad_kernel<BM, BN, WM, WN, VEC, 0>), grid, dim3(WM * WN * 64), 0, stream, a);
        else if (scm == 1) hipLaunchKernelGGL((conv_wgrad_kernel<BM, BN, WM, WN, VEC, 1>), grid, dim3(WM * WN * 64), 0, stream, a);
        else hipLaunchKernelGGL((conv_wgrad_kernel<BM, BN, WM, WN, VEC, 2>), grid, dim3(WM * WN * 64), 0, stream, a);
    }
}
template <int BM, int BN, int WM, int WN>
void launch_wgrad(hipStream_t stream, const WgradArgs& a, dim3 grid, bool vec, int scm) {
    if (vec) launch_wgrad2<BM, BN, WM, WN, true>(stream, a, grid, scm);
    else launch_wgrad2<BM, BN, WM, WN, false>(stream, a, grid, scm);
}
// ... 136 lines not shown
    }

    const WgTile t = pick_wg_tile(p->Cin, p->Cout);
    dim3 grid(ceil_div(p->Cin, t.BM), ceil_div(p->Cout, t.BN), p->KH * p->KW * splits);
    a.xp = nullptr; a.dyp = nullptr;
    const size_t partial_floats = (splits > 1) ? (size_t)splits * wsize : 0;
    if (wgrad_planes_shape_ok(p) && p->workspace != nullptr && (((uintptr_t)p->workspace | (uintptr_t)p->x | (uintptr_t)p->dy | (uintptr_t)p->in_scale | (uintptr_t)p->out_scale | (uintptr_t)p->x_pieces | (uintptr_t)p->dy_pieces) & 15) == 0 &&
        p->workspace_floats >= partial_floats + wgrad_planes_x_floats(p) + wgrad_planes_dy_floats(p)) {
        IGAN_REQUIRE((p->x_pieces == nullptr && p->dy_pieces == nullptr) || planes_mode() == 1, "conv2d_wgrad: the two-piece fp16 form writes its own images (one scale per channel): x_pieces / dy_pieces must be NULL");
        IGAN_REQUIRE(p->x_pieces == nullptr || p->x_pieces_bytes == wgrad_planes_x_floats(p) * 4, "conv2d_wgrad: x_pieces is not the image of this x (x_pieces_bytes != N*H*W*Cin*6)");
        IGAN_REQUIRE(p->dy_pieces == nullptr || p->dy_pieces_bytes == wgrad_planes_dy_floats(p) * 4, "conv2d_wgrad: dy_pieces is not the image of this dy (dy_pieces_bytes != N*OH*OW*Cout*6)");
        const unsigned short* xp = reinterpret_cast<const unsigned short*>(p->x_pieces);
        const unsigned short* dyp = reinterpret_cast<const unsigned short*>(p->dy_pieces);
        if (xp == nullptr) {
            unsigned short* own = reinterpret_cast<unsigned short*>(p->workspace + partial_floats);
            if (planes_mode() == 2) launch_col_image(stream, p->x, p->in_scale, own, p->N * p->H * p->W, p->H * p->W, p->Cin, p->x_colmax);
            else launch_piece_image(stream, p->x, p->in_scale, own, p->N * p->H * p->W, p->H * p->W, p->Cin);
            xp = own;
        }
        if (dyp == nullptr) {
            unsigned short* own = reinterpret_cast<unsigned short*>(p->workspace + partial_floats + wgrad_planes_x_floats(p));
            if (planes_mode() == 2) launch_col_image(stream, p->dy, p->out_scale, own, p->N * p->OH * p->OW, p->OH * p->OW, p->Cout, p->dy_colmax);
            else launch_piece_image(stream, p->dy, p->out_scale, own, p->N * p->OH * p->OW, p->OH * p->OW, p->Cout);
            dyp = own;
        }
        a.xp = xp; a.dyp = dyp;
        if (planes_mode() == 2) hipLaunchKernelGGL((conv_wgrad_planes_kernel<2>), grid, dim3(512), 0, stream, a);
        else hipLaunchKernelGGL((conv_wgrad_planes_kernel<3>), grid, dim3(512), 0, stream, a);
        IGAN_LAUNCH_CHECK("conv2d_wgrad (piece form) launch");
        if (splits > 1) {
            const int total = (int)wsize;
            const int rg = std::min(ceil_div(total, 256), 2048);
            hipLaunchKernelGGL(plain_reduce_kernel, dim3(rg), dim3(256), 0, stream, (const float*)p->workspace, p->dw, total, splits, p->alpha);
            IGAN_LAUNCH_CHECK("conv2d_wgrad reduce launch");
        }
        return IGAN_OK;
    }
    const bool vec = a.vecA && a.vecB && (a.in_scale == nullptr || a.vecSA) && (a.out_scale == nullptr || a.vecSB);
    const int scm = (a.in_scale && a.out_scale) ? 1 : ((a.in_scale || a.out_scale) ? 2 : 0);
    const bool long_axis = (long long)p->OH * p->OW >= 128LL * 128LL;
    if (t.BM == 128 && t.BN == 128 && eight_waves("IGAN_WGRAD_8WAVE") && !long_axis && scm == 0) launch_wgrad<128, 128, 2, 4>(stream, a, grid, vec, scm);
    else if (t.BM == 128 && t.BN == 128) launch_wgrad<128, 128, 2, 2>(stream, a, grid, vec, scm);
    else if (t.BM == 128 && t.BN == 32) launch_wgrad<128, 32, 4, 1>(stream, a, grid, vec, scm);
    else launch_wgrad<32, 128, 1, 4>(stream, a, grid, vec, scm);
    IGAN_LAUNCH_CHECK("conv2d_wgrad launch");
    if (splits > 1) {
        const int total = (int)wsize;
        const int rg = std::min(ceil_div(total, 256), 2048);
        hipLaunchKernelGGL(plain_reduce_kernel, dim3(rg), dim3(256), 0, stream, (const float*)p->workspace, p->dw, total, splits, p->alpha);
        IGAN_LAUNCH_CHECK("conv2d_wgrad reduce launch");
    }
    return IGAN_OK;
}

static int f16_window_read(unsigned long long (&v)[4], int reset) {
    using namespace igan;
    if (hipMemcpyFromSymbol(&v[0], HIP_SYMBOL(g_f16_below_window), 8) != hipSuccess || hipMemcpyFromSymbol(&v[1], HIP_SYMBOL(g_f16_imaged), 8) != hipSuccess ||
        hipMemcpyFromSymbol(&v[2], HIP_SYMBOL(g_f16_below_window_cols), 8) != hipSuccess || hipMemcpyFromSymbol(&v[3], HIP_SYMBOL(g_f16_imaged_cols), 8) != hipSuccess) return IGAN_ERR_HIP;
    if (reset) {
        const unsigned long long z = 0ull;
        if (hipMemcpyToSymbol(HIP_SYMBOL(g_f16_below_window), &z, 8) != hipSuccess || hipMemcpyToSymbol(HIP_SYMBOL(g_f16_imaged), &z, 8) != hipSuccess ||
            hipMemcpyToSymbol(HIP_SYMBOL(g_f16_below_window_cols), &z, 8) != hipSuccess || hipMemcpyToSymbol(HIP_SYMBOL(g_f16_imaged_cols), &z, 8) != hipSuccess) return IGAN_ERR_HIP;
    }
    return IGAN_OK;
}
extern "C" int igan_debug_f16_window(unsigned long long* below, unsigned long long* imaged, int reset) {
    unsigned long long v[4] = {0ull, 0ull, 0ull, 0ull};
    if (int rc = f16_window_read(v, reset)) return rc;
    if (below) *below = v[0] + v[2];
    if (imaged) *imaged = v[1] + v[3];
    return IGAN_OK;
}
extern "C" int igan_debug_f16_window_by_kind(unsigned long long* out4, int reset) {
    using namespace igan;
    IGAN_REQUIRE(out4 != nullptr, "debug_f16_window_by_kind: null argument");
    unsigned long long v[4] = {0ull, 0ull, 0ull, 0ull};
    if (int rc = f16_window_read(v, reset)) return rc;
    for (int i = 0; i < 4; i++) out4[i] = v[i];
    return IGAN_OK;
}

extern "C" int igan_conv_piece_form(void) { return planes_mode(); }

extern "C" size_t igan_colmax_floats(int N, int HW, int C) {
    using namespace igan;
    if (planes_mode() != 2 || N < 1 || HW < 1 || C < 16 || C > 1024 || (C & (C - 1)) != 0) return 0;
    if ((long long)N * HW < wgrad_min_rows()) return 0;
    return 4 + (size_t)H_COLBLOCKS * C;
}

extern "C" size_t igan_filter_image_bytes(int KH, int KW, int Cin, int Cout) {
    using namespace igan;
    if (!planes_enabled() || KH < 1 || KW < 1 || Cin < 1 || Cout < 1 || KH * KW == 1 || Cin % BK != 0 || (long long)KH * KW * Cin < 1152) return 0;
    if ((long long)KH * KW * Cin * Cout * 6 >= 0x7FFFFF00LL) return 0;
    if (planes_mode() == 2) {
        if (!pow2(Cin / PK) || Cin / PK > 64 || KH * KW > 9 || Cout % 4 != 0) return 0;
        return filter_part_bytes((size_t)KH * KW, (size_t)Cout, (size_t)Cin);
    }
    return (size_t)KH * KW * Cin * Cout * 6;
}

extern "C" int igan_filter_image(igan_stream_t stream_, const float* w, void* out, int KH, int KW, int Cin, int Cout, int w_transposed) {
    using namespace igan;
    IGAN_REQUIRE(w != nullptr && out != nullptr, "filter_image: null buffer");
    IGAN_REQUIRE(igan_filter_image_bytes(KH, KW, Cin, Cout) != 0, "filter_image: igan_filter_image_bytes() says this process / filter takes none");
    IGAN_REQUIRE(((((uintptr_t)w) | ((uintptr_t)out)) & 15) == 0, "filter_image: w and out must be 16-byte aligned");
    launch_filter_image((hipStream_t)stream_, w, reinterpret_cast<unsigned short*>(out), w_transposed != 0, KH * KW, KW, Cout, Cin);
    IGAN_LAUNCH_CHECK("filter_image launch");
    return IGAN_OK;
}

extern "C" int igan_conv_pieces_wanted(int KH, int KW, int Cin, int Cout) {
    using namespace igan;
    return (planes_enabled() && KH * KW > 1 && Cin >= 128 && Cout >= 128 && Cin % 32 == 0 && Cout % 32 == 0) ? 1 : 0;
}

extern "C" int igan_pieces_image_ok(int N, int HW, int C) {
    using namespace igan;
    return (planes_mode() == 1 && C >= 128 && C % 32 == 0 && (long long)N * HW >= 2048 && (long long)N * HW * C * 6 < 0x7FFFFF00LL) ? 1 : 0;
}

extern "C" int igan_to_pieces(igan_stream_t stream_, const float* x, const float* scale, void* out, int N, int HW, int C) {
    using namespace igan;
    IGAN_REQUIRE(x != nullptr && out != nullptr, "to_pieces: null buffer");
    IGAN_REQUIRE(N >= 1 && HW >= 1 && C >= 16 && C % 16 == 0, "to_pieces: C must be a positive multiple of 16");
    IGAN_REQUIRE((((uintptr_t)x | (uintptr_t)scale | (uintptr_t)out) & 15) == 0, "to_pieces: buffers must be 16-byte aligned");
    IGAN_REQUIRE((long long)N * HW * C * 6 < 0x7FFFFF00LL, "to_pieces: image too large (32-bit offsets)");
    if (planes_mode() != 1) return igan::fail(IGAN_ERR_UNSUPPORTED, "to_pieces: only the bf16-piece form (IGAN_CONV_PLANES=1) takes caller-written images (igan_pieces_image_ok() says so)");
    launch_piece_image((hipStream_t)stream_, x, scale, reinterpret_cast<unsigned short*>(out), N * HW, HW, C);
    IGAN_LAUNCH_CHECK("to_pieces launch");
    return IGAN_OK;
}
```

### inclusivegan_amd/csrc/igan_common.h

```cpp
#pragma once
#include <hip/hip_runtime.h>
#include <cstdarg>
#include <cstdio>
#include <cstdint>
#include "../../include/igan_hip.h"

namespace igan {

char* error_buffer();
int fail(int code, const char* fmt, ...);

inline int check_hip(hipError_t e, const char* what) {
    if (e == hipSuccess) return IGAN_OK;
    return fail(IGAN_ERR_HIP, "%s: %s", what, hipGetErrorName(e));
}

#define IGAN_REQUIRE(cond, ...)                                   \
    do {                                                          \
        if (!(cond)) return ::igan::fail(IGAN_ERR_INVALID_ARGUMENT, __VA_ARGS__); \
    } while (0)

#define IGAN_LAUNCH_CHECK(what)                                   \
    do {                                                          \
        hipError_t e__ = hipGetLastError();                       \
        if (e__ != hipSuccess) return ::igan::check_hip(e__, what); \
    } while (0)

#define IGAN_HIP_CHECK(call, what)                                \
    do {                                                          \
        hipError_t e__ = (call);                                  \
        if (e__ != hipSuccess) return ::igan::check_hip(e__, what); \
    } while (0)

bool dense_small_ok(int M, int K, int N, const void* x, const void* w, bool wt);
bool dense_small_fits(long long M, long long K, long long N, long long ldx);
int dense_small_rows(int M);
void dense_small_launch(hipStream_t stream, const igan_dense_params& a);
void dense_small(hipStream_t stream, const float* x, const float* w, float* y, int M, int K, int N, bool wt, float alpha);
bool dense_small_wgrad_ok(int M, int N, const void* dy, const void* dw);
void dense_small_wgrad(hipStream_t stream, const float* x, const float* dy, float* dw, int M, int K, int N, float alpha);

int thin_conv_kind(const igan_conv2d_params* p);
void thin_conv(hipStream_t stream, const igan_conv2d_params* p, int kind);
int thin_wgrad_kind(const igan_conv2d_wgrad_params* p);
size_t thin_wgrad_workspace(const igan_conv2d_wgrad_params* p, int kind);
void thin_wgrad(hipStream_t stream, const igan_conv2d_wgrad_params* p, int kind);

inline int ceil_div(int a, int b) { return (a + b - 1) / b; }
inline long long ceil_div_ll(long long a, long long b) { return (a + b - 1) / b; }

}
```

### inclusivegan_amd/hip_ops.py

```python
import ctypes
import os
from collections import namedtuple

import numpy as np
import torch

from . import _abi

CL = torch.channels_last


def _stream():
    return ctypes.c_void_p(torch.cuda.current_stream().cuda_stream)


def _ptr(t):
    return ctypes.c_void_p(t.data_ptr()) if t is not None else ctypes.c_void_p(0)


def _require_cuda_f32(*ts):
    for t in ts:
        if t is None:
            continue
        if not t.is_cuda:
# ... 229 lines not shown
class _BiasGradFn(torch.autograd.Function):

    @staticmethod
    def forward(ctx, dx, axis, size_b, step_b):
        ctx.shape = dx.shape
        ctx.axis = axis
        return bias_grad_raw(dx, size_b, step_b)

    @staticmethod
    def backward(ctx, d_db):
        view = [1] * len(ctx.shape)
        view[ctx.axis] = -1
        return d_db.view(*view).expand(ctx.shape), None, None, None


class FusedBiasActFn(torch.autograd.Function):
    @staticmethod
    def forward(ctx, x, b, axis, act_idx, alpha, gain, ref_kind, zero_2nd):
        xd, size_b, step_b = _bias_layout(x, axis)
        y = fused_bias_act_raw(xd, b, None, 0, act_idx, alpha, gain, size_b, step_b)
        ctx.save_for_backward(xd if ref_kind == 'x' else y)
        ctx.cfg = (axis, act_idx, alpha, gain, size_b, step_b, zero_2nd)
        ctx.has_b = b is not None
        return y

    @staticmethod
    def backward(ctx, dy):
        (ref,) = ctx.saved_tensors
        axis, act_idx, alpha, gain, size_b, step_b, zero_2nd = ctx.cfg
        dx = _FbaGradFn.apply(dy, None, ref, axis, act_idx, alpha, gain, size_b, step_b, zero_2nd)
        db = _BiasGradFn.apply(dx, axis, size_b, step_b) if (ctx.has_b and _needed(ctx, 1)) else None
        return (dx, db) + (None,) * 6


class FusedBiasActSmoothFn(torch.autograd.Function):

    @staticmethod
    def forward(ctx, x, b, axis, act_idx, alpha, gain, ref_kind):
        xd, size_b, step_b = _bias_layout(x, axis)
        y = fused_bias_act_raw(xd, b, None, 0, act_idx, alpha, gain, size_b, step_b)
        ctx.cfg = (axis, act_idx, alpha, gain, size_b, step_b, ref_kind)
        ctx.has_b = b is not None
        ctx.save_for_backward(xd, y, b)
        return y

    @staticmethod
    def backward(ctx, dy):
        xd, y, b = ctx.saved_tensors
        axis, act_idx, alpha, gain, size_b, step_b, ref_kind = ctx.cfg
        ref = (xd if ref_kind == 'x' else y).detach()
        if torch.is_grad_enabled():
            recv = xd
            if ref_kind != 'x' and b is not None:
                view = [1] * xd.dim(); view[axis] = -1
                recv = xd + b.view(*view)
            dx = _FbaGradFn.apply(dy, None, ref, axis, act_idx, alpha, gain, size_b, step_b, False, recv)
        else:
            dx = fused_bias_act_raw(_match_layout(dy, ref), None, ref, 1, act_idx, alpha, gain, size_b, step_b)
        db = _BiasGradFn.apply(dx, axis, size_b, step_b) if (ctx.has_b and _needed(ctx, 1)) else None
        return (dx, db) + (None,) * 5



def _rows_c(x):
    if x.dim() == 4 and x.is_contiguous(memory_format=CL) and x.shape[1] % 4 == 0:
        return x.shape[0] * x.shape[2] * x.shape[3], x.shape[1]
    if x.dim() == 2 and x.is_contiguous() and x.shape[1] % 4 == 0:
        return x.shape[0], x.shape[1]
    return None


def bias_act_noise_fwd_raw(x, noise, strength, b, act_idx, alpha, gain):
    if _is_meta(x):
        return torch.empty_like(x)
    lib = _abi.get_plugin()
    _require_cuda_f32(x, noise, strength, b)
    rows, c = _rows_c(x)
    y = torch.empty_like(x)
    _abi.check(lib.igan_bias_act_noise_fwd(_stream(), _ptr(x), _ptr(noise), _ptr(strength), _ptr(b), _ptr(y),
                                           rows, c, act_idx, float(alpha), float(gain)))
    return y


def bias_act_noise_bwd_raw(dy, y, noise, act_idx, alpha, gain, want_db):
    lib = _abi.get_plugin()
    _require_cuda_f32(dy, y, noise)
    rows, c = _rows_c(y)
    dy = _match_layout(dy, y)
    dx = torch.empty_like(y)
    ws = torch.empty((int(lib.igan_bias_act_noise_workspace_floats(rows, c)),), device=y.device, dtype=torch.float32)
    db = torch.empty((c,), device=y.device, dtype=torch.float32) if want_db else None
    ds = torch.empty((), device=y.device, dtype=torch.float32) if noise is not None else None
    _abi.check(lib.igan_bias_act_noise_bwd(_stream(), _ptr(dy), _ptr(y), _ptr(noise), _ptr(dx), _ptr(db), _ptr(ds), _ptr(ws),
                                           rows, c, act_idx, float(alpha), float(gain)))
    return dx, db, ds


class BiasActNoiseFn(torch.autograd.Function):

    @staticmethod
    def forward(ctx, x, b, noise, strength, act_idx, alpha, gain):
        _mark_inputs(ctx, x, b, noise, strength, act_idx, alpha, gain)
        y = bias_act_noise_fwd_raw(x, noise, strength, b, act_idx, alpha, gain)
        ctx.save_for_backward(y, noise)
        ctx.cfg = (act_idx, alpha, gain)
        ctx.has_b = b is not None
        return y

    @staticmethod
    def backward(ctx, dy):
        y, noise = ctx.saved_tensors
        act_idx, alpha, gain = ctx.cfg
        need_b = ctx.has_b and _needed(ctx, 1)
        need_s = noise is not None and _needed(ctx, 3)
        if torch.is_grad_enabled():
            c = y.shape[1]
            dx = _FbaGradFn.apply(dy, None, y, 1, act_idx, alpha, gain, c, 1, True)
            db = _BiasGradFn.apply(dx, 1, c, 1) if need_b else None
            ds = (dx * noise.reshape(_noise_view(y))).sum() if need_s else None
            return dx, db, None, ds, None, None, None
        dx, db, ds = bias_act_noise_bwd_raw(dy, y, noise, act_idx, alpha, gain, need_b)
        return dx, db, None, (ds if need_s else None), None, None, None


def _noise_view(y):
    return (y.shape[0], 1, y.shape[2], y.shape[3]) if y.dim() == 4 else (y.shape[0], 1)


def bias_act_noise(x, b, noise, strength, act_idx, alpha, gain):
    if _is_meta(x):
        return torch.empty_like(x)
    if x.dim() in (2, 4) and x.shape[1] % 4 == 0:
        x = nhwc(x) if x.dim() == 4 else x.contiguous()
        if noise is not None:
            noise = noise.expand(_noise_view(x)).contiguous()
        return BiasActNoiseFn.apply(x, b, noise, strength, act_idx, alpha, gain)
    if noise is not None:
        x = x + noise * strength
    return FusedBiasActFn.apply(x, b, 1, act_idx, alpha, gain, 'y', True)



ConvGeom = namedtuple('ConvGeom', 'kh kw stride up pad_y pad_x alpha', defaults=(1.0,))

_plan_cache = {}
_wplan_cache = {}

launch_log = None
stamp_log = None
shape_log = None


class StampLog:

    def __init__(self, device, capacity=16384):
        self.stamps = torch.zeros((2 * capacity,), device=device, dtype=torch.int64)
        self.acc = torch.zeros((capacity,), device=device, dtype=torch.int64)
        self.entries = []
        self.shapes = []
        self.capacity = capacity
        self._folded = 0
        self.folds = {}

    def bracket(self, name, flops, launch, shape=None):
        i = len(self.entries)
        if i >= self.capacity:
            raise RuntimeError('StampLog: capacity exceeded')
        lib = _abi.get_plugin()
        self.entries.append((name, flops))
        self.shapes.append(shape)
        _abi.check(lib.igan_stamp(_stream(), ctypes.c_void_p(self.stamps.data_ptr() + 16 * i)))
        launch()
        _abi.check(lib.igan_stamp(_stream(), ctypes.c_void_p(self.stamps.data_ptr() + 16 * i + 8)))

    def fold(self):
# ... 22 lines not shown
    e0 = torch.cuda.Event(enable_timing=True)
    e1 = torch.cuda.Event(enable_timing=True)
    e0.record()
    launch()
    e1.record()
    shape_log.append((kind, key, flops, splits, e0, e1))


def conv_flops(n, h, w, cin, oh, ow, cout, geom):
    up = geom.up
    pairs = 0
    for py in range(up):
        for px in range(up):
            qh = (oh - py + up - 1) // up
            qw = (ow - px + up - 1) // up
            ky0 = (geom.pad_y - py * geom.stride) % up
            kx0 = (geom.pad_x - px * geom.stride) % up
            nky = (geom.kh - ky0 + up - 1) // up if ky0 < geom.kh else 0
            nkx = (geom.kw - kx0 + up - 1) // up if kx0 < geom.kw else 0
            pairs += qh * qw * nky * nkx
    return 2.0 * n * pairs * cin * cout


PIECES_SHARE = os.environ.get('IGAN_PIECES_SHARE', '1') != '0'

_pieces_rule = {}


def pieces_wanted(geom, cin, cout):
    if not PIECES_SHARE:
        return False
    key = (geom.kh, geom.kw, int(cin), int(cout))
    hit = _pieces_rule.get(key)
    if hit is None:
        hit = _pieces_rule[key] = bool(_abi.get_plugin().igan_conv_pieces_wanted(*key))
    return hit


class PieceImage:
    __slots__ = ('buf', 'nbytes')

    def __init__(self, buf, nbytes):
        self.buf, self.nbytes = buf, nbytes

    def data_ptr(self):
        return self.buf.data_ptr()


def to_pieces(x, scale=None):
    if not PIECES_SHARE or _is_meta(x) or x.dim() != 4:
        return None
    n, c, h, w = x.shape
    if not _abi.get_plugin().igan_pieces_image_ok(int(n), int(h * w), int(c)):
        return None
    x = nhwc(x)
    if scale is not None:
        scale = scale.contiguous()
    out = torch.empty((n * h * w * c * 6 // 4,), device=x.device, dtype=torch.float32)
    if (x.data_ptr() | out.data_ptr() | (scale.data_ptr() if scale is not None else 0)) & 15:
        return None
    launch = lambda: _abi.check(_abi.get_plugin().igan_to_pieces(_stream(), _ptr(x), (_ptr(scale) if scale is not None else None), _ptr(out), n, h * w, c))
    if stamp_log is not None:
        stamp_log.bracket('to_planes_kernel (shared image)', 0.0, launch, shape='%-12s N%-3d %3dx%-3d C%-4d' % ('pieces', n, h, w, c))
    else:
        launch()
    return PieceImage(out, n * h * w * c * 6)


_colmax_floats = {}
COLMAX_SHARE = os.environ.get('IGAN_COLMAX_SHARE', '1') != '0'


def colmax_buffer(x, want=True):
    if not (want and COLMAX_SHARE) or _is_meta(x) or x.dim() != 4:
        return None
    n, c, h, w = x.shape
    key = (int(n), int(h * w), int(c))
    fl = _colmax_floats.get(key)
    if fl is None:
        fl = _colmax_floats[key] = int(_abi.get_plugin().igan_colmax_floats(*key))
    if fl == 0:
        return None
    return torch.empty((fl,), device=x.device, dtype=torch.float32)


_filter_bytes = {}
FILTER_CACHE = os.environ.get('IGAN_FILTER_CACHE', '1') != '0'


def mark_constant(w):
    w._igan_constant = True
    return w


def _constant_filter_image(lib, w, geom, cin, cout, w_transposed):
    if not (FILTER_CACHE and getattr(w, '_igan_constant', False)):
        return None
    key = (geom.kh, geom.kw, int(cin), int(cout))
    nbytes = _filter_bytes.get(key)
    if nbytes is None:
        nbytes = _filter_bytes[key] = int(lib.igan_filter_image_bytes(*key))
    if nbytes == 0 or (w.data_ptr() & 15):
        return None
    cache = getattr(w, '_igan_filter_images', None)
    if cache is None or cache[0] != w._version:
        if cache is not None:
            w._igan_filter_keepalive = getattr(w, '_igan_filter_keepalive', []) + list(cache[1].values())
        cache = (w._version, {})
        w._igan_filter_images = cache
    img = cache[1].get((key, bool(w_transposed)))
    if img is None:
        if torch.cuda.is_current_stream_capturing():
            return None
        img = torch.empty(((nbytes + 3) // 4,), device=w.device, dtype=torch.float32)
        _abi.check(lib.igan_filter_image(_stream(), _ptr(w), _ptr(img), geom.kh, geom.kw, int(cin), int(cout), 1 if w_transposed else 0))
        cache[1][(key, bool(w_transposed))] = img
    return PieceImage(img, nbytes)


def conv2d_raw(x, w, geom, out_hw, cout, w_transposed=False, in_scale=None, out_scale=None, bias=None, act=None, noise=None, strength=None, x_pieces=None, colmax=None):
    if _is_meta(x):
        return torch.empty((x.shape[0], cout, out_hw[0], out_hw[1]), device='meta')
    lib = _abi.get_plugin()
    _require_cuda_f32(x, w, in_scale, out_scale, bias)
    x = nhwc(x)
    w = w.contiguous()
    n, cin, h, wd = x.shape
    oh, ow = out_hw
    y = empty_nchw(n, cout, oh, ow, x)
    if bias is not None:
        bias = bias.contiguous()
    if in_scale is not None:
        in_scale = in_scale.contiguous()
    if out_scale is not None:
        out_scale = out_scale.contiguous()
    p = _abi.Conv2DParams(
        x=x.data_ptr(), w=w.data_ptr(), y=y.data_ptr(),
        in_scale=(in_scale.data_ptr() if in_scale is not None else None),
        out_scale=(out_scale.data_ptr() if out_scale is not None else None),
        workspace=None, workspace_floats=0,
        N=n, H=h, W=wd, Cin=cin, OH=oh, OW=ow, Cout=cout,
        KH=geom.kh, KW=geom.kw, stride=geom.stride, up=geom.up,
        pad_y=geom.pad_y, pad_x=geom.pad_x,
        w_transposed=1 if w_transposed else 0, splits=1, alpha=float(geom.alpha),
        bias=(bias.data_ptr() if bias is not None else None), act=(int(act[0]) if act is not None else 0),
        act_alpha=(float(act[1]) if act is not None else 0.0), act_gain=(float(act[2]) if act is not None else 1.0))
    if x_pieces is not None:
        p.x_pieces = x_pieces.data_ptr()
        p.x_pieces_bytes = x_pieces.nbytes
    if colmax is not None:
        p.x_colmax = colmax.data_ptr()
    wimg = _constant_filter_image(lib, w, geom, cin, cout, w_transposed)
    if wimg is not None:
        p.w_pieces = wimg.data_ptr()
        p.w_pieces_bytes = wimg.nbytes
    if noise is not None:
        noise = noise.contiguous()
        _require_cuda_f32(noise, strength)
        if act is None or strength is None or noise.numel() not in (oh * ow, n * oh * ow):
            raise ValueError('conv2d: noise needs the fused epilogue, a strength scalar and [N or 1, 1, OH, OW] values')
        p.noise = noise.data_ptr(); p.noise_strength = strength.data_ptr(); p.noise_bcast = 1 if (noise.numel() == oh * ow and n > 1) else 0
    key = (n, h, wd, cin, oh, ow, cout, geom, act is not None, bool(w_transposed), in_scale is not None, out_scale is not None)
    plan = _plan_cache.get(key)
    if plan is None:
        splits = ctypes.c_int(1)
        sliced = ctypes.c_int(0)
        wsf = ctypes.c_size_t(0)
        _abi.check(lib.igan_conv2d_plan(ctypes.byref(p), ctypes.byref(splits), ctypes.byref(sliced), ctypes.byref(wsf)))
        plan = (splits.value, wsf.value, sliced.value)
        _plan_cache[key] = plan
    ws = None
    if plan[1] > 0:
        ws = torch.empty((plan[1],), device=x.device, dtype=torch.float32)
        p.workspace = ws.data_ptr()
        p.workspace_floats = plan[1]
    if plan[0] > 1:
        p.splits = plan[0]
        p.sliced_tiles = plan[2]
    if stamp_log is not None:
        buf = ctypes.create_string_buffer(128)
        _abi.check(lib.igan_conv2d_kernel_name(ctypes.byref(p), buf, 128))
        kind = ('dgrad' if w_transposed else 'fwd') + ('+scale' if (in_scale is not None or out_scale is not None) else '') + ('+act' if act is not None else '')
        stamp_log.bracket(buf.value.decode(), conv_flops(n, h, wd, cin, oh, ow, cout, geom),
                          lambda: _abi.check(lib.igan_conv2d(_stream(), ctypes.byref(p))),
                          shape='%-12s N%-3d %3dx%-3d C%-4d -> %3dx%-3d C%-4d k%d s%d u%d splits %d' % (kind, n, h, wd, cin, oh, ow, cout, geom.kh, geom.stride, geom.up, plan[0]))
        return y
    if launch_log is not None:
        buf = ctypes.create_string_buffer(128)
        _abi.check(lib.igan_conv2d_kernel_name(ctypes.byref(p), buf, 128))
        e0 = torch.cuda.Event(enable_timing=True)
        e1 = torch.cuda.Event(enable_timing=True)
        e0.record()
        _abi.check(lib.igan_conv2d(_stream(), ctypes.byref(p)))
        e1.record()
        launch_log.append((buf.value.decode(), conv_flops(n, h, wd, cin, oh, ow, cout, geom), plan[0], e0, e1))
        return y
    if shape_log is not None:
        kind = ('dgrad' if w_transposed else 'fwd') + ('+s' if in_scale is not None else '')
        _shape_logged(kind, key, conv_flops(n, h, wd, cin, oh, ow, cout, geom), plan[0],
                      lambda: _abi.check(lib.igan_conv2d(_stream(), ctypes.byref(p))))
        return y
    _abi.check(lib.igan_conv2d(_stream(), ctypes.byref(p)))
    return y


def conv2d_wgrad_raw(x, dy, geom, in_scale=None, out_scale=None, x_pieces=None, dy_pieces=None, x_colmax=None, dy_colmax=None):
    lib = _abi.get_plugin()
    _require_cuda_f32(x, dy, in_scale, out_scale)
    x = nhwc(x)
    dy = nhwc(dy)
    n, cin, h, wd = x.shape
    n2, cout, oh, ow = dy.shape
    if n2 != n:
        raise ValueError('conv2d_wgrad: batch mismatch')
    dw = torch.empty((geom.kh, geom.kw, cin, cout), device=x.device, dtype=torch.float32)
    if in_scale is not None:
        in_scale = in_scale.contiguous()
    if out_scale is not None:
        out_scale = out_scale.contiguous()
    p = _abi.Conv2DWgradParams(
        x=x.data_ptr(), dy=dy.data_ptr(), dw=dw.data_ptr(),
        in_scale=(in_scale.data_ptr() if in_scale is not None else None),
        out_scale=(out_scale.data_ptr() if out_scale is not None else None),
        workspace=None, workspace_floats=0,
        N=n, H=h, W=wd, Cin=cin, OH=oh, OW=ow, Cout=cout,
        KH=geom.kh, KW=geom.kw, stride=geom.stride, up=geom.up,
        pad_y=geom.pad_y, pad_x=geom.pad_x, splits=1, alpha=float(geom.alpha))
    if x_pieces is not None:
        p.x_pieces = x_pieces.data_ptr()
        p.x_pieces_bytes = x_pieces.nbytes
    if dy_pieces is not None:
        p.dy_pieces = dy_pieces.data_ptr()
        p.dy_pieces_bytes = dy_pieces.nbytes
    if x_colmax is not None:
# ... 47 lines not shown

    @staticmethod
    def backward(ctx, dy):
        x, w = ctx.saved_tensors
        dx = dw = None
        if _needed(ctx, 0):
            dx = ConvDgradFn.apply(dy, w, ctx.geom, ctx.in_hw)
        if _needed(ctx, 1):
            dw = ConvWgradFn.apply(x, dy, ctx.geom)
        return dx, dw, None, None


class ConvDgradFn(torch.autograd.Function):

    @staticmethod
    def forward(ctx, dy, w, geom, in_hw):
        ctx.save_for_backward(dy, w)
        ctx.geom = geom
        ctx.out_hw = (dy.shape[2], dy.shape[3])
        return conv2d_raw(dy, w, dgrad_geom(geom), in_hw, w.shape[2], w_transposed=True)

    @staticmethod
    def backward(ctx, ddx):
        dy, w = ctx.saved_tensors
        d_dy = d_w = None
        if _needed(ctx, 0):
            d_dy = Conv2dFn.apply(ddx, w, ctx.geom, ctx.out_hw)
        if _needed(ctx, 1):
            d_w = ConvWgradFn.apply(ddx, dy, ctx.geom)
        return d_dy, d_w, None, None


class ConvWgradFn(torch.autograd.Function):

    @staticmethod
    def forward(ctx, x, dy, geom):
        ctx.save_for_backward(x, dy)
        ctx.geom = geom
        return conv2d_wgrad_raw(x, dy, geom)

    @staticmethod
    def backward(ctx, ddw):
        x, dy = ctx.saved_tensors
        d_x = d_dy = None
        if _needed(ctx, 0):
            d_x = ConvDgradFn.apply(dy, ddw, ctx.geom, (x.shape[2], x.shape[3]))
        if _needed(ctx, 1):
            d_dy = Conv2dFn.apply(x, ddw, ctx.geom, (dy.shape[2], dy.shape[3]))
        return d_x, d_dy, None


class ConvBiasActFn(torch.autograd.Function):

    @staticmethod
    def forward(ctx, x, w, b, geom, out_hw, act_idx, alpha, gain):
        share = pieces_wanted(geom, x.shape[1], w.shape[3]) and ctx.needs_input_grad[1]
        xp = to_pieces(x) if share else None
        xcm = colmax_buffer(x, share)
        y = conv2d_raw(x, w, geom, out_hw, w.shape[3], bias=b, act=(act_idx, alpha, gain), x_pieces=xp, colmax=xcm)
        ctx.save_for_backward(x, w, y)
        ctx.xp, ctx.xcm = xp, xcm
        ctx.geom, ctx.cfg = geom, (act_idx, alpha, gain)
        ctx.in_hw = (x.shape[2], x.shape[3])
        ctx.has_b = b is not None
        return y

    @staticmethod
    def backward(ctx, dy):
        x, w, y = ctx.saved_tensors
        act_idx, alpha, gain = ctx.cfg
        need_x, need_w = _needed(ctx, 0), _needed(ctx, 1)
        need_b = ctx.has_b and _needed(ctx, 2)
        dx = dw = db = None
        if torch.is_grad_enabled():
            c = y.shape[1]
            dxp = _FbaGradFn.apply(dy, None, y, 1, act_idx, alpha, gain, c, 1, True)
            if need_b:
                db = _BiasGradFn.apply(dxp, 1, c, 1)
            if need_x:
                dx = ConvDgradFn.apply(dxp, w, ctx.geom, ctx.in_hw)
            if need_w:
                dw = ConvWgradFn.apply(x, dxp, ctx.geom)
            return dx, dw, db, None, None, None, None, None
        dxp, db, _ = bias_act_noise_bwd_raw(dy, y, None, act_idx, alpha, gain, need_b)
        share = pieces_wanted(ctx.geom, x.shape[1], y.shape[1]) and need_x and need_w
        dyp = to_pieces(dxp) if share else None
        dycm = colmax_buffer(dxp, share)
        if need_x:
            dx = conv2d_raw(dxp, w, dgrad_geom(ctx.geom), ctx.in_hw, w.shape[2], w_transposed=True, x_pieces=dyp, colmax=dycm)
        if need_w:
            dw = conv2d_wgrad_raw(x, dxp, ctx.geom, x_pieces=ctx.xp, dy_pieces=dyp, x_colmax=ctx.xcm, dy_colmax=dycm)
        return dx, dw, (db if need_b else None), None, None, None, None, None


def conv_bias_act_fusable(x, cout, act_idx):
    return (not _is_meta(x)) and x.is_cuda and x.dim() == 4 and x.shape[1] > 4 and cout % 4 == 0 and act_idx in (1, 2, 3) and _CONV_EPILOGUE


_CONV_EPILOGUE = os.environ.get('IGAN_CONV_EPILOGUE', '1') != '0'


def conv2d(x, w, geom, out_hw):
    return Conv2dFn.apply(x, w, geom, out_hw)


def matmul(x, w, alpha=1.0):
    n, cin = x.shape
    y = Conv2dFn.apply(x.reshape(n, cin, 1, 1), w.reshape(1, 1, cin, w.shape[1]), ConvGeom(1, 1, 1, 1, 0, 0, float(alpha)), (1, 1))
    return y.reshape(n, w.shape[1])



def scale_dot_raw(a, b, s=None, want_scaled=False):
    lib = _abi.get_plugin()
    _require_cuda_f32(a, b, s)
    a = nhwc(a)
    b = nhwc(b)
    n, c, h, w = a.shape
    dot = torch.empty((n, c), device=a.device, dtype=torch.float32)
    ws = torch.empty((int(lib.igan_scale_dot_workspace_floats(n, h * w, c)),), device=a.device, dtype=torch.float32)
    if s is not None:
        s = s.contiguous()
    _abi.check(lib.igan_scale_dot(_stream(), _ptr(a), _ptr(b), _ptr(s), _ptr(b) if want_scaled else ctypes.c_void_p(0),
                                  _ptr(dot), _ptr(ws), n, h * w, c))
    return dot, (b if want_scaled else None)


class ModConv2dFn(torch.autograd.Function):

    @staticmethod
    def forward(ctx, x, w, s, d, geom, out_hw):
        share = pieces_wanted(geom, x.shape[1], w.shape[3]) and ctx.needs_input_grad[1]
        xp = to_pieces(x, s) if share else None
        xcm = colmax_buffer(x, share)
        y = conv2d_raw(x, w, geom, out_hw, w.shape[3], in_scale=s, out_scale=d, x_pieces=xp, colmax=xcm)
        ctx.save_for_backward(x, w, s, d, y)
        ctx.xp, ctx.xcm = xp, xcm
        ctx.geom = geom
        ctx.out_hw = out_hw
        return y

    @staticmethod
    def backward(ctx, dy):
        x, w, s, d, y = ctx.saved_tensors
        geom = ctx.geom
        need_x, need_w, need_s, need_d = [_needed(ctx, i) for i in range(4)]
        in_hw = (x.shape[2], x.shape[3])
        if torch.is_grad_enabled():
            dx = dw = ds = dd = None
            if (not need_w) and d is not None and _MODCONV_GRAD_FN and x.shape[1] % 4 == 0 and y.shape[1] % 4 == 0:
                dx, ds, dd = ModConvGradFn.apply(dy, x, w, s, d, y, geom, in_hw, ctx.out_hw)
                return (dx if need_x else None), None, (ds if need_s else None), (dd if need_d else None), None, None
            dyd = dy * d[:, :, None, None] if d is not None else dy
            if need_x or need_s:
                dxs = ConvDgradFn.apply(dyd, w, geom, in_hw)
                if need_x:
                    dx = dxs * s[:, :, None, None]
                if need_s:
                    ds = (dxs * x).sum(dim=(2, 3))
            if need_w or (need_d and d is not None):
                xs = x * s[:, :, None, None]
                if need_w:
                    dw = ConvWgradFn.apply(xs, dyd, geom)
                if need_d and d is not None:
                    dd = (dy * Conv2dFn.apply(xs, w, geom, ctx.out_hw)).sum(dim=(2, 3))
            return dx, dw, ds, dd, None, None
        dx = dw = ds = dd = None
        dy = nhwc(dy)
        share = pieces_wanted(geom, x.shape[1], y.shape[1]) and (need_x or need_s) and need_w
        dyp = to_pieces(dy, d) if share else None
        dycm = colmax_buffer(dy, share)
        if need_x or need_s:
            dxs = conv2d_raw(dy, w, dgrad_geom(geom), in_hw, w.shape[2], w_transposed=True, in_scale=d, x_pieces=dyp, colmax=dycm)
            if x.shape[1] % 4 == 0:
                ds, dx = scale_dot_raw(x, dxs, s, want_scaled=need_x)
                if not need_s:
                    ds = None
            else:
                if need_s:
                    ds = (x * dxs).sum(dim=(2, 3))
                if need_x:
                    dx = dxs * s[:, :, None, None]
        if need_w:
            dw = conv2d_wgrad_raw(x, dy, geom, in_scale=s, out_scale=d, x_pieces=ctx.xp, dy_pieces=dyp, x_colmax=ctx.xcm, dy_colmax=dycm)
        if need_d and d is not None:
            if y.shape[1] % 4 == 0:
                dd = scale_dot_raw(dy, y)[0] / d
            else:
                dd = (dy * y).sum(dim=(2, 3)) / d
        return dx, dw, ds, dd, None, None


_MODCONV_GRAD_FN = os.environ.get('IGAN_MODCONV_GRAD_FN', '1') != '0'


class ModConvGradFn(torch.autograd.Function):

    @staticmethod
    def forward(ctx, dy, x, w, s, d, y, geom, in_hw, out_hw):
        dy = nhwc(dy)
        t = conv2d_raw(dy, w, dgrad_geom(geom), in_hw, w.shape[2], w_transposed=True, in_scale=d)
        ds, _ = scale_dot_raw(x, t, None)
        dx = t * s[:, :, None, None]
        dd = scale_dot_raw(dy, y)[0] / d
        ctx.save_for_backward(dy, x, w, s, d, y, t)
        ctx.geom, ctx.in_hw, ctx.out_hw = geom, in_hw, out_hw
        return dx, ds, dd

    @staticmethod
    def backward(ctx, g_dx, g_ds, g_dd):
        if torch.is_grad_enabled():
            raise NotImplementedError('modulated conv: third-order gradients are not built')
        dy, x, w, s, d, y, t = ctx.saved_tensors
        geom = ctx.geom
        need_dy, need_x, need_w, need_s, need_d = [_needed(ctx, i) for i in range(5)]
        g_dy = g_x = g_w = g_s = g_d = None
        if g_dx is not None or g_ds is not None:
            if g_dx is not None:
                g_t = nhwc(g_dx) * s[:, :, None, None]
                if g_ds is not None:
                    g_t = torch.addcmul(g_t, x, g_ds[:, :, None, None])
            else:
                g_t = x * g_ds[:, :, None, None]
            if need_dy or need_d:
                g_dy = conv2d_raw(g_t, w, geom, ctx.out_hw, w.shape[3], out_scale=d)
                if need_d:
                    g_d = scale_dot_raw(g_dy, dy)[0] / d
            if need_w:
                g_w = conv2d_wgrad_raw(g_t, dy, geom, out_scale=d)
            if need_s and g_dx is not None:
                g_s = scale_dot_raw(g_dx, t)[0]
            if need_x and g_ds is not None:
                g_x = t * g_ds[:, :, None, None]
        if g_dd is not None:
            g_dd = g_dd.contiguous()
            if need_x or need_s:
                g_xs = conv2d_raw(dy, w, dgrad_geom(geom), ctx.in_hw, w.shape[2], w_transposed=True, in_scale=g_dd)
                gs2, gx2 = scale_dot_raw(x, g_xs, s, want_scaled=need_x)
                if need_s:
                    g_s = gs2 if g_s is None else g_s + gs2
                if need_x:
                    g_x = gx2 if g_x is None else g_x + gx2
            if need_w:
                gw2 = conv2d_wgrad_raw(x, dy, geom, in_scale=s, out_scale=g_dd)
                g_w = gw2 if g_w is None else g_w + gw2
            if need_dy:
                gdy2 = y * (g_dd / d)[:, :, None, None]
                g_dy = gdy2 if g_dy is None else g_dy + gdy2
        return g_dy, g_x, g_w, g_s, g_d, None, None, None, None


def bias_act_noise_bwd_dd_raw(dy, y, noise, strength, b, d, act_idx, alpha, gain):
    lib = _abi.get_plugin()
    _require_cuda_f32(dy, y, noise, strength, b, d)
    y = nhwc(y)
    dy = nhwc(dy)
    n, c, h, w = y.shape
    dx = torch.empty_like(y)
    ws = torch.empty((int(lib.igan_bias_act_noise_dd_workspace_floats(n, h * w, c)),), device=y.device, dtype=torch.float32)
    db = torch.empty((c,), device=y.device, dtype=torch.float32)
    ds = torch.empty((), device=y.device, dtype=torch.float32) if noise is not None else None
    dd = torch.empty((n, c), device=y.device, dtype=torch.float32)
    bcast = 1 if (noise is not None and noise.numel() == h * w and n > 1) else 0
    _abi.check(lib.igan_bias_act_noise_bwd_dd(_stream(), _ptr(dy), _ptr(y), _ptr(noise), _ptr(strength), _ptr(b), _ptr(d.contiguous()), _ptr(dx), _ptr(db),
                                              _ptr(ds), _ptr(dd), _ptr(ws), bcast, n, h * w, c, act_idx, float(alpha), float(gain)))
    return dx, db, ds, dd


class ModConvBanFn(torch.autograd.Function):

    @staticmethod
    def forward(ctx, x, w, s, d, b, noise, strength, geom, out_hw, act_idx, alpha, gain):
        _mark_inputs(ctx, x, w, s, d, b, noise, strength, geom, out_hw, act_idx, alpha, gain)
        share = pieces_wanted(geom, x.shape[1], w.shape[3]) and ctx.needs_input_grad[1]
        xp = to_pieces(x, s) if share else None
        xcm = colmax_buffer(x, share)
        y = conv2d_raw(x, w, geom, out_hw, w.shape[3], in_scale=s, out_scale=d, bias=b, act=(act_idx, alpha, gain), noise=noise, strength=strength, x_pieces=xp, colmax=xcm)
        ctx.save_for_backward(x, w, s, d, b, noise, strength, y)
        ctx.xp, ctx.xcm = xp, xcm
        ctx.geom, ctx.out_hw, ctx.cfg = geom, out_hw, (act_idx, alpha, gain)
        return y

    @staticmethod
    def backward(ctx, dy):
        if torch.is_grad_enabled():
            raise NotImplementedError('fused synthesis layer: second-order gradients go through ModConv2dFn + BiasActNoiseFn (hip_ops.second_order())')
        x, w, s, d, b, noise, strength, y = ctx.saved_tensors
        act_idx, alpha, gain = ctx.cfg
        geom = ctx.geom
        need_x, need_w, need_s, need_d, need_b = [_needed(ctx, i) for i in range(5)]
        need_st = noise is not None and _needed(ctx, 6)
        dxp, db, dst, dd = bias_act_noise_bwd_dd_raw(dy, y, noise, strength, b, d, act_idx, alpha, gain)
        dx = dw = ds = None
        in_hw = (x.shape[2], x.shape[3])
        share = pieces_wanted(geom, x.shape[1], y.shape[1]) and (need_x or need_s) and need_w
        dyp = to_pieces(dxp, d) if share else None
        dycm = colmax_buffer(dxp, share)
        if need_x or need_s:
            dxs = conv2d_raw(dxp, w, dgrad_geom(geom), in_hw, w.shape[2], w_transposed=True, in_scale=d, x_pieces=dyp, colmax=dycm)
            ds, dx = scale_dot_raw(x, dxs, s, want_scaled=need_x)
            if not need_s:
                ds = None
        if need_w:
            dw = conv2d_wgrad_raw(x, dxp, geom, in_scale=s, out_scale=d, x_pieces=ctx.xp, dy_pieces=dyp, x_colmax=ctx.xcm, dy_colmax=dycm)
        return dx, dw, ds, (dd if need_d else None), (db if need_b else None), None, (dst if need_st else None), None, None, None, None, None


def modconv_ban_fusable(x, w, d, b, noise, act_idx):
    return (_MODCONV_BAN and _second_order_depth == 0 and not _is_meta(x) and x.is_cuda and d is not None and b is not None
            and act_idx in (1, 3) and x.shape[1] % 32 == 0 and w.shape[3] % 32 == 0 and x.shape[1] >= 32 and 32 <= w.shape[3] <= 1024)


_MODCONV_BAN = os.environ.get('IGAN_MODCONV_BAN', '1') != '0'


def modconv_composite(x, w, s, d, geom, out_hw):
    y = Conv2dFn.apply(x * s[:, :, None, None], w, geom, out_hw)
    if d is not None:
        y = y * d[:, :, None, None]
    return y



def _row_major(t):
    if t.dim() != 2 or t.stride(1) != 1 or t.stride(0) % 4 != 0 or t.stride(0) < t.shape[1] or t.data_ptr() % 16 != 0:
        t = t.contiguous()
    return t


def dense_small_raw(x, w, w_transposed=False, alpha=1.0, prologue=_abi.DENSE_PRO_NONE, x2=None, pro_scale=0.0,
                    epilogue=_abi.DENSE_EPI_SCALE, bias=None, bias_scale=1.0, add_const=0.0, eps=0.0, e1=None, e2=None,
                    want_colsum=False):
    lib = _abi.get_plugin()
    _require_cuda_f32(x, w, x2, bias, e1, e2)
    x = _row_major(x)
    w = w.contiguous()
    m, k = x.shape
    n = w.shape[0] if w_transposed else w.shape[1]
    y = torch.empty((m, n), device=x.device, dtype=torch.float32)
    colsum = torch.empty((n,), device=x.device, dtype=torch.float32) if want_colsum else None
    x2 = x2.contiguous() if x2 is not None else None
    e1 = e1.contiguous() if e1 is not None else None
    e2 = e2.contiguous() if e2 is not None else None
    bias = bias.contiguous() if bias is not None else None
    p = _abi.DenseParams(x=x.data_ptr(), x2=_ptr(x2), w=w.data_ptr(), y=y.data_ptr(), bias=_ptr(bias), e1=_ptr(e1), e2=_ptr(e2),
                         colsum=_ptr(colsum), ldx=x.stride(0), ldy=n, M=m, K=k, N=n, w_transposed=1 if w_transposed else 0,
                         prologue=prologue, epilogue=epilogue, alpha=float(alpha), pro_scale=float(pro_scale),
                         bias_scale=float(bias_scale), add_const=float(add_const), eps=float(eps))
    _abi.check(lib.igan_dense_small(_stream(), ctypes.byref(p)))
    return (y, colsum) if want_colsum else y


def dense_small_wgrad_raw(a, b, alpha=1.0, pro_a=_abi.DENSE_PRO_NONE, pro_b=_abi.DENSE_PRO_NONE, b2=None, pro_scale=0.0):
    lib = _abi.get_plugin()
    _require_cuda_f32(a, b, b2)
    a = _row_major(a)
    b = b.contiguous()
    b2 = b2.contiguous() if b2 is not None else None
    m, k = a.shape
    n = b.shape[1]
    dw = torch.empty((k, n), device=a.device, dtype=torch.float32)
    p = _abi.DenseWgradParams(a=a.data_ptr(), b=b.data_ptr(), b2=_ptr(b2), dw=dw.data_ptr(), lda=a.stride(0), M=m, K=k, N=n,
                              pro_a=pro_a, pro_b=pro_b, alpha=float(alpha), pro_scale=float(pro_scale))
    _abi.check(lib.igan_dense_small_wgrad(_stream(), ctypes.byref(p)))
    return dw


def sumsq_taps_raw(w):
    lib = _abi.get_plugin()
    _require_cuda_f32(w)
    w = w.contiguous()
    out = torch.empty(tuple(w.shape[2:]), device=w.device, dtype=torch.float32)
    _abi.check(lib.igan_sumsq_taps(_stream(), _ptr(w), _ptr(out), w.shape[0] * w.shape[1], out.numel()))
    return out


def bcast_mul_taps_raw(w, v, scale):
    lib = _abi.get_plugin()
    _require_cuda_f32(w, v)
    w = w.contiguous()
    v = v.contiguous()
    out = torch.empty_like(w)
# ... 704 lines not shown
```

Baseline: 355.5.

## Fuse fp16 row-image production into bias-act-noise backward for dgrad conv

The bias/act/noise backward kernels now optionally also write a two-piece fp16 row image of the scaled gradient, plus per-row inverse scales and column maxima, which the following dgrad convolution consumes as pre-split input. This is meant to remove the separate conversion/splitting pass inside the planes-type conv kernel and the extra read of the gradient tensor. It is enabled by default through an environment switch and only when the conv dispatch picks the planes kernel and the shape fits. In exchange it adds more register pressure and extra stores in the elementwise kernel, and the loop now runs partial iterations so that the warp shuffles stay uniform.

```diff
diff --git a/include/igan_hip.h b/include/igan_hip.h
--- a/include/igan_hip.h
+++ b/include/igan_hip.h
@@ -71,6 +71,14 @@
 int igan_bias_act_noise_bwd_dd(igan_stream_t stream, const float* dy, const float* y, const float* noise, const float* strength,
                                const float* b, const float* dscale, float* dx, float* db, float* dstrength, float* dd,
                                float* workspace, int noise_bcast, int N, int HW, int C, int act, float alpha, float gain);
+
+int igan_bias_act_noise_image_ok(int N, int HW, int C);
+int igan_bias_act_noise_bwd_rows(igan_stream_t stream, const float* dy, const float* y, const float* noise,
+                                 float* dx, float* db, float* dstrength, float* workspace,
+                                 int rows, int C, int act, float alpha, float gain, const float* dscale, int HW, void* rows_out, float* colmax);
+int igan_bias_act_noise_bwd_dd_rows(igan_stream_t stream, const float* dy, const float* y, const float* noise, const float* strength,
+                                    const float* b, const float* dscale, float* dx, float* db, float* dstrength, float* dd,
+                                    float* workspace, int noise_bcast, int N, int HW, int C, int act, float alpha, float gain, void* rows_out, float* colmax);
 
 typedef struct igan_conv2d_params {
     const float* x;
@@ -100,6 +108,8 @@
     float* x_colmax;
     const void* w_pieces;
     size_t w_pieces_bytes;
+    const void* x_rows;
+    size_t x_rows_bytes;
 } igan_conv2d_params;
 
 int igan_conv2d_plan(const igan_conv2d_params* p, int* splits, int* sliced_tiles, size_t* workspace_floats);
@@ -139,6 +149,8 @@
 size_t igan_filter_image_bytes(int KH, int KW, int Cin, int Cout);
 int igan_filter_image(igan_stream_t stream, const float* w, void* out, int KH, int KW, int Cin, int Cout, int w_transposed);
 size_t igan_colmax_floats(int N, int HW, int C);
+size_t igan_row_image_bytes(int N, int HW, int C);
+int igan_row_image(igan_stream_t stream, const float* x, const float* scale, void* out, int N, int HW, int C, float* colmax);
 int igan_debug_f16_window(unsigned long long* below, unsigned long long* imaged, int reset);
 int igan_debug_f16_window_by_kind(unsigned long long* out4, int reset);
 
diff --git a/inclusivegan_amd/_abi.py b/inclusivegan_amd/_abi.py
--- a/inclusivegan_amd/_abi.py
+++ b/inclusivegan_amd/_abi.py
@@ -49,6 +49,7 @@
         ('x_pieces', ctypes.c_void_p), ('x_pieces_bytes', ctypes.c_size_t),
         ('x_colmax', ctypes.c_void_p),
         ('w_pieces', ctypes.c_void_p), ('w_pieces_bytes', ctypes.c_size_t),
+        ('x_rows', ctypes.c_void_p), ('x_rows_bytes', ctypes.c_size_t),
     ]
 
     def __init__(self, *args, **kwargs):
@@ -129,6 +130,9 @@
     'igan_bias_act_noise_dd_workspace_floats': (ctypes.c_size_t, [_I, _I, _I]),
     'igan_bias_act_noise_bwd_dd': (_I, [_P, _P, _P, _P, _P, _P, _P, _P, _P, _P, _P, _P, _I, _I, _I, _I, _I, _F, _F]),
     'igan_bias_act_noise_bwd': (_I, [_P, _P, _P, _P, _P, _P, _P, _P, _I, _I, _I, _F, _F]),
+    'igan_bias_act_noise_image_ok': (_I, [_I, _I, _I]),
+    'igan_bias_act_noise_bwd_rows': (_I, [_P, _P, _P, _P, _P, _P, _P, _P, _I, _I, _I, _F, _F, _P, _I, _P, _P]),
+    'igan_bias_act_noise_bwd_dd_rows': (_I, [_P, _P, _P, _P, _P, _P, _P, _P, _P, _P, _P, _P, _I, _I, _I, _I, _I, _F, _F, _P, _P]),
     'igan_conv2d_plan': (_I, [ctypes.POINTER(Conv2DParams), ctypes.POINTER(_I), ctypes.POINTER(_I), ctypes.POINTER(_SZ)]),
     'igan_conv2d': (_I, [_P, ctypes.POINTER(Conv2DParams)]),
     'igan_conv2d_kernel_name': (_I, [ctypes.POINTER(Conv2DParams), ctypes.c_char_p, _I]),
@@ -137,6 +141,8 @@
     'igan_conv2d_wgrad': (_I, [_P, ctypes.POINTER(Conv2DWgradParams)]),
     'igan_debug_f16_window_by_kind': (_I, [_P, _I]),
     'igan_colmax_floats': (ctypes.c_size_t, [_I, _I, _I]),
+    'igan_row_image_bytes': (ctypes.c_size_t, [_I, _I, _I]),
+    'igan_row_image': (_I, [_P, _P, _P, _P, _I, _I, _I, _P]),
     'igan_filter_image_bytes': (ctypes.c_size_t, [_I, _I, _I, _I]),
     'igan_filter_image': (_I, [_P, _P, _P, _I, _I, _I, _I, _I]),
     'igan_to_pieces': (_I, [_P, _P, _P, _P, _I, _I, _I]),
diff --git a/inclusivegan_amd/csrc/bias_act_noise.hip b/inclusivegan_amd/csrc/bias_act_noise.hip
--- a/inclusivegan_amd/csrc/bias_act_noise.hip
+++ b/inclusivegan_amd/csrc/bias_act_noise.hip
@@ -1,6 +1,61 @@
 #include "igan_common.h"
+#include "row_image.h"
 
 namespace {
+
+struct RowImgArgs {
+    const float* scale;
+    unsigned short* out;
+    float* rowinv;
+    float* colmax;
+    unsigned long long* below;
+    unsigned long long* imaged;
+    int HW;
+    long long total;
+};
+
+__device__ __forceinline__ void image_row_quad(const RowImgArgs& im, const float4& d, const float4& sc, int r, int col, int cvt, int C, bool live, float4& cm, int& below) {
+    float v[4] = {d.x, d.y, d.z, d.w};
+    if (im.scale != nullptr) { v[0] *= sc.x; v[1] *= sc.y; v[2] *= sc.z; v[3] *= sc.w; }
+    float m = 0.0f;
+    float av[4];
+#pragma unroll
+    for (int i = 0; i < 4; i++) { av[i] = fabsf(v[i]); m = fmaxf(m, av[i]); }
+    if (live) { cm.x = fmaxf(cm.x, av[0]); cm.y = fmaxf(cm.y, av[1]); cm.z = fmaxf(cm.z, av[2]); cm.w = fmaxf(cm.w, av[3]); }
+    for (int o = 1; o < cvt; o <<= 1) m = fmaxf(m, __shfl_xor(m, o));
+    const float S = scale_from_amax(m);
+    if (live && col == 0) im.rowinv[r] = inv_scale_from_amax(m);
+    unsigned short pc[2][4];
+#pragma unroll
+    for (int i = 0; i < 4; i++) {
+        unsigned short o[2];
+        const float vs = v[i] * S;
+        split2_row(vs, o);
+        pc[0][i] = o[0]; pc[1][i] = o[1];
+        below += live ? below_window(vs) : 0;
+    }
+    const unsigned a0 = pc[0][0] | ((unsigned)pc[0][1] << 16), a1 = pc[0][2] | ((unsigned)pc[0][3] << 16);
+    const unsigned b0 = pc[1][0] | ((unsigned)pc[1][1] << 16), b1 = pc[1][2] | ((unsigned)pc[1][3] << 16);
+    const bool odd = (col & 1) != 0;
+    const unsigned g0 = __shfl_xor(odd ? a0 : b0, 1), g1 = __shfl_xor(odd ? a1 : b1, 1);
+    const uint4 w = odd ? make_uint4(g0, g1, b0, b1) : make_uint4(a0, a1, g0, g1);
+    if (live) *reinterpret_cast<uint4*>(im.out + row_image_index((size_t)r, 4 * (col & ~1), C, odd ? 1 : 0)) = w;
+}
+
+__device__ __forceinline__ void image_colmax(const RowImgArgs& im, float4* red, const float4& cm, int col, int cvt, int rl, int C) {
+    __syncthreads();
+    red[threadIdx.x] = cm;
+    __syncthreads();
+    if ((int)threadIdx.x < cvt) {
+        float4 t = red[threadIdx.x];
+        for (int j = 1; j < rl; j++) {
+            const float4 u = red[threadIdx.x + j * cvt];
+            t.x = fmaxf(t.x, u.x); t.y = fmaxf(t.y, u.y); t.z = fmaxf(t.z, u.z); t.w = fmaxf(t.w, u.w);
+        }
+        *reinterpret_cast<float4*>(im.colmax + 4 + (size_t)blockIdx.x * C + (size_t)col * 4) = t;
+    }
+    if (blockIdx.x == 0 && threadIdx.x == 0) im.colmax[0] = (float)gridDim.x;
+}
 
 struct BanArgs {
     const float* x;
@@ -46,7 +101,8 @@
     }
 }
 
-__global__ __launch_bounds__(256) void ban_bwd_kernel(BanArgs a) {
+template <bool IMG>
+__global__ __launch_bounds__(256) void ban_bwd_kernel(BanArgs a, RowImgArgs im) {
     __shared__ float4 red[256];
     __shared__ float reds[256];
     const int cv = a.C >> 2;
@@ -63,9 +119,11 @@
     float4* dx4 = reinterpret_cast<float4*>(a.y);
     float4 accb = make_float4(0.f, 0.f, 0.f, 0.f);
     float accs = 0.f;
+    float4 cm = make_float4(0.f, 0.f, 0.f, 0.f);
+    int below = 0;
     if (active) {
-        for (int rb = r0 + lane_r; rb < r1; rb += 4 * rl) {
-            float4 g[4], yy[4];
+        for (int rb = r0 + lane_r; IMG ? (rb - lane_r < r1) : (rb < r1); rb += 4 * rl) {
+            float4 g[4], yy[4], sc[4];
             float nz[4];
 #pragma unroll
             for (int u = 0; u < 4; u++) {
@@ -74,20 +132,22 @@
                 g[u] = dy4[i];
                 yy[u] = y4[i];
                 nz[u] = a.noise ? a.noise[r] : 0.f;
+                if constexpr (IMG) sc[u] = im.scale ? reinterpret_cast<const float4*>(im.scale)[(size_t)(r / im.HW) * cv + col] : make_float4(1.f, 1.f, 1.f, 1.f);
             }
 #pragma unroll
             for (int u = 0; u < 4; u++) {
                 const int r = rb + u * rl;
+                float4 d;
+                d.x = __fmul_rn(act_bwd(a.act, g[u].x, yy[u].x, a.alpha), a.gain);
+                d.y = __fmul_rn(act_bwd(a.act, g[u].y, yy[u].y, a.alpha), a.gain);
+                d.z = __fmul_rn(act_bwd(a.act, g[u].z, yy[u].z, a.alpha), a.gain);
+                d.w = __fmul_rn(act_bwd(a.act, g[u].w, yy[u].w, a.alpha), a.gain);
                 if (r < r1) {
-                    float4 d;
-                    d.x = act_bwd(a.act, g[u].x, yy[u].x, a.alpha) * a.gain;
-                    d.y = act_bwd(a.act, g[u].y, yy[u].y, a.alpha) * a.gain;
-                    d.z = act_bwd(a.act, g[u].z, yy[u].z, a.alpha) * a.gain;
-                    d.w = act_bwd(a.act, g[u].w, yy[u].w, a.alpha) * a.gain;
                     dx4[(long long)r * cv + col] = d;
                     accb.x += d.x; accb.y += d.y; accb.z += d.z; accb.w += d.w;
                     accs += nz[u] * ((d.x + d.y) + (d.z + d.w));
                 }
+                if constexpr (IMG) image_row_quad(im, d, sc[u], min(r, r1 - 1), col, cvt, a.C, r < r1, cm, below);
             }
         }
     }
@@ -113,6 +173,13 @@
         if (threadIdx.x == 0) a.partial[(size_t)blockIdx.x * (a.C + 1) + a.C] = (reds[0] + reds[1]) + (reds[2] + reds[3]);
     } else if (!a.noise && blockIdx.y == 0 && threadIdx.x == 0) {
         a.partial[(size_t)blockIdx.x * (a.C + 1) + a.C] = 0.f;
+    }
+    if constexpr (IMG) {
+        if (im.colmax != nullptr) image_colmax(im, red, cm, col, cvt, rl, a.C);
+        count_window(below, im.below);
+#ifndef IGAN_NO_WINDOW_COUNT
+        if (blockIdx.x == 0 && threadIdx.x == 0) atomicAdd(im.imaged, (unsigned long long)im.total);
+#endif
     }
 }
 
@@ -142,7 +209,8 @@
     }
 }
 
-__global__ __launch_bounds__(256) void ban_bwd_dd_kernel(BanArgs a, const float* __restrict__ strength_p, int HW, int bps) {
+template <bool IMG>
+__global__ __launch_bounds__(256) void ban_bwd_dd_kernel(BanArgs a, const float* __restrict__ strength_p, int HW, int bps, RowImgArgs im) {
     __shared__ float4 red[256];
     __shared__ float4 red2[256];
     __shared__ float reds[256];
@@ -166,8 +234,11 @@
     if (active && a.b) bb = *reinterpret_cast<const float4*>(a.b + 4 * col);
     float4 accb = make_float4(0.f, 0.f, 0.f, 0.f), accd = make_float4(0.f, 0.f, 0.f, 0.f);
     float accs = 0.f;
+    float4 cm = make_float4(0.f, 0.f, 0.f, 0.f), sc = make_float4(1.f, 1.f, 1.f, 1.f);
+    int below = 0;
+    if constexpr (IMG) { if (active && im.scale) sc = reinterpret_cast<const float4*>(im.scale)[(size_t)n * cv + col]; }
     if (active) {
-        for (int rb = r0 + lane_r; rb < r1; rb += 4 * rl) {
+        for (int rb = r0 + lane_r; IMG ? (rb - lane_r < r1) : (rb < r1); rb += 4 * rl) {
             float4 g[4], yy[4];
             float nz[4];
 #pragma unroll
@@ -181,12 +252,13 @@
 #pragma unroll
             for (int u = 0; u < 4; u++) {
                 const int r = rb + u * rl;
+                float4 d;
+                d.x = __fmul_rn(act_bwd(a.act, g[u].x, yy[u].x, a.alpha), a.gain);
+                d.y = __fmul_rn(act_bwd(a.act, g[u].y, yy[u].y, a.alpha), a.gain);
+                d.z = __fmul_rn(act_bwd(a.act, g[u].z, yy[u].z, a.alpha), a.gain);
+                d.w = __fmul_rn(act_bwd(a.act, g[u].w, yy[u].w, a.alpha), a.gain);
+                if constexpr (IMG) image_row_quad(im, d, sc, min(r, r1 - 1), col, cvt, a.C, r < r1, cm, below);
                 if (r < r1) {
-                    float4 d;
-                    d.x = act_bwd(a.act, g[u].x, yy[u].x, a.alpha) * a.gain;
-                    d.y = act_bwd(a.act, g[u].y, yy[u].y, a.alpha) * a.gain;
-                    d.z = act_bwd(a.act, g[u].z, yy[u].z, a.alpha) * a.gain;
-                    d.w = act_bwd(a.act, g[u].w, yy[u].w, a.alpha) * a.gain;
                     dx4[(long long)r * cv + col] = d;
                     accb.x += d.x; accb.y += d.y; accb.z += d.z; accb.w += d.w;
                     accs += nz[u] * ((d.x + d.y) + (d.z + d.w));
@@ -224,6 +296,13 @@
         if ((threadIdx.x & 63) == 0) reds[threadIdx.x >> 6] = s;
         __syncthreads();
         if (threadIdx.x == 0) a.partial[(size_t)blockIdx.x * W + a.C] = (reds[0] + reds[1]) + (reds[2] + reds[3]);
+    }
+    if constexpr (IMG) {
+        if (im.colmax != nullptr) image_colmax(im, red, cm, col, cvt, rl, a.C);
+        count_window(below, im.below);
+#ifndef IGAN_NO_WINDOW_COUNT
+        if (blockIdx.x == 0 && threadIdx.x == 0) atomicAdd(im.imaged, (unsigned long long)im.total);
+#endif
     }
 }
 
@@ -294,9 +373,30 @@
     return (size_t)N * ban_dd_bps(N, HW, C) * (size_t)(2 * C + 1);
 }
 
-extern "C" int igan_bias_act_noise_bwd_dd(igan_stream_t stream_, const float* dy, const float* y, const float* noise, const float* strength,
-                                          const float* b, const float* dscale, float* dx, float* db, float* dstrength, float* dd,
-                                          float* workspace, int noise_bcast, int N, int HW, int C, int act, float alpha, float gain) {
+namespace {
+
+bool ban_image_ok(int N, int HW, int C, int blocks) {
+    return N >= 1 && HW >= 1 && C >= 32 && C <= 256 && igan_row_image_bytes(N, HW, C) != 0 && blocks <= H_COLBLOCKS;
+}
+
+int ban_image_args(const char* who, RowImgArgs& im, const float* dscale, void* rows_out, float* colmax, int N, int HW, int C, int blocks) {
+    IGAN_REQUIRE(rows_out != nullptr, "%s: null image buffer", who);
+    if (!ban_image_ok(N, HW, C, blocks)) return igan::fail(IGAN_ERR_UNSUPPORTED, "%s: no row image is written for N %d, HW %d, C %d (igan_bias_act_noise_image_ok() says so)", who, N, HW, C);
+    IGAN_REQUIRE((((uintptr_t)rows_out | (uintptr_t)colmax | (uintptr_t)dscale) & 15) == 0, "%s: the image, colmax and the scale must be 16-byte aligned", who);
+    IGAN_REQUIRE(colmax == nullptr || igan_colmax_floats(N, HW, C) != 0, "%s: colmax given, but igan_colmax_floats() says this process / tensor takes none", who);
+    im.scale = dscale;
+    im.out = reinterpret_cast<unsigned short*>(rows_out);
+    im.rowinv = row_image_rowinv(rows_out, (size_t)N * HW, (size_t)C);
+    im.colmax = colmax;
+    im.HW = HW;
+    im.total = (long long)N * HW * C;
+    if (int rc = igan::f16_row_counters(&im.below, &im.imaged)) return rc;
+    return IGAN_OK;
+}
+
+int ban_bwd_dd_impl(igan_stream_t stream_, const float* dy, const float* y, const float* noise, const float* strength,
+                    const float* b, const float* dscale, float* dx, float* db, float* dstrength, float* dd,
+                    float* workspace, int noise_bcast, int N, int HW, int C, int act, float alpha, float gain, bool image, void* rows_out, float* colmax) {
     using namespace igan;
     IGAN_REQUIRE(dy && y && dx && workspace && dscale && dd, "bias_act_noise_bwd_dd: null buffer");
     IGAN_REQUIRE((noise == nullptr) || (strength != nullptr && dstrength != nullptr), "bias_act_noise_bwd_dd: noise given without strength / dstrength");
@@ -309,11 +409,59 @@
     BanArgs a{dy, y, noise, nullptr, b, dx, workspace, noise_bcast ? -1 : N * HW, C, act, alpha, gain};
     const int bps = ban_dd_bps(N, HW, C);
     dim3 grid(N * bps, ceil_div(C / 4, 256));
-    hipLaunchKernelGGL(ban_bwd_dd_kernel, grid, dim3(256), 0, (hipStream_t)stream_, a, strength, HW, bps);
+    RowImgArgs im{};
+    if (image) {
+        if (int rc = ban_image_args("bias_act_noise_bwd_dd_rows", im, dscale, rows_out, colmax, N, HW, C, N * bps)) return rc;
+        hipLaunchKernelGGL(ban_bwd_dd_kernel<true>, grid, dim3(256), 0, (hipStream_t)stream_, a, strength, HW, bps, im);
+    } else
+        hipLaunchKernelGGL(ban_bwd_dd_kernel<false>, grid, dim3(256), 0, (hipStream_t)stream_, a, strength, HW, bps, im);
     hipLaunchKernelGGL(ban_dd_final_kernel, dim3(ceil_div(C + 1, 16), 1 + N), dim3(256), 0, (hipStream_t)stream_,
                        (const float*)workspace, dscale, db, noise ? dstrength : nullptr, dd, N, bps, C);
     IGAN_LAUNCH_CHECK("bias_act_noise_bwd_dd launch");
     return IGAN_OK;
+}
+
+int ban_bwd_impl(igan_stream_t stream_, const float* dy, const float* y, const float* noise,
+                 float* dx, float* db, float* dstrength, float* workspace,
+                 int rows, int C, int act, float alpha, float gain, bool image, const float* dscale, int HW, void* rows_out, float* colmax) {
+    using namespace igan;
+    IGAN_REQUIRE(dy && y && dx && workspace, "bias_act_noise_bwd: null buffer");
+    IGAN_REQUIRE((noise == nullptr) || (dstrength != nullptr), "bias_act_noise_bwd: noise given without dstrength");
+    if (int rc = ban_check("bias_act_noise_bwd", rows, C, act, gain)) return rc;
+    IGAN_REQUIRE((((uintptr_t)dy | (uintptr_t)y | (uintptr_t)dx) & 15) == 0, "bias_act_noise_bwd: buffers must be 16-byte aligned");
+    BanArgs a{dy, y, noise, nullptr, nullptr, dx, workspace, rows, C, act, alpha, gain};
+    const int blocks = ban_blocks(rows, C);
+    dim3 grid(blocks, ceil_div(C / 4, 256));
+    RowImgArgs im{};
+    if (image) {
+        IGAN_REQUIRE(HW >= 1 && rows % HW == 0, "bias_act_noise_bwd_rows: rows must be a whole number of samples of HW pixels");
+        if (int rc = ban_image_args("bias_act_noise_bwd_rows", im, dscale, rows_out, colmax, rows / HW, HW, C, blocks)) return rc;
+        hipLaunchKernelGGL(ban_bwd_kernel<true>, grid, dim3(256), 0, (hipStream_t)stream_, a, im);
+    } else
+        hipLaunchKernelGGL(ban_bwd_kernel<false>, grid, dim3(256), 0, (hipStream_t)stream_, a, im);
+    hipLaunchKernelGGL(ban_final_kernel, dim3(ceil_div(C + 1, 16)), dim3(256), 0, (hipStream_t)stream_,
+                       (const float*)workspace, db, noise ? dstrength : nullptr, blocks, C);
+    IGAN_LAUNCH_CHECK("bias_act_noise_bwd launch");
+    return IGAN_OK;
+}
+
+}
+
+extern "C" int igan_bias_act_noise_bwd_dd(igan_stream_t stream_, const float* dy, const float* y, const float* noise, const float* strength,
+                                          const float* b, const float* dscale, float* dx, float* db, float* dstrength, float* dd,
+                                          float* workspace, int noise_bcast, int N, int HW, int C, int act, float alpha, float gain) {
+    return ban_bwd_dd_impl(stream_, dy, y, noise, strength, b, dscale, dx, db, dstrength, dd, workspace, noise_bcast, N, HW, C, act, alpha, gain, false, nullptr, nullptr);
+}
+
+extern "C" int igan_bias_act_noise_bwd_dd_rows(igan_stream_t stream_, const float* dy, const float* y, const float* noise, const float* strength,
+                                               const float* b, const float* dscale, float* dx, float* db, float* dstrength, float* dd,
+                                               float* workspace, int noise_bcast, int N, int HW, int C, int act, float alpha, float gain, void* rows_out, float* colmax) {
+    return ban_bwd_dd_impl(stream_, dy, y, noise, strength, b, dscale, dx, db, dstrength, dd, workspace, noise_bcast, N, HW, C, act, alpha, gain, true, rows_out, colmax);
+}
+
+extern "C" int igan_bias_act_noise_image_ok(int N, int HW, int C) {
+    if (N < 1 || HW < 1 || C < 32 || C > 256 || (long long)N * HW > INT32_MAX) return 0;
+    return (ban_image_ok(N, HW, C, ban_blocks(N * HW, C)) && ban_image_ok(N, HW, C, N * ban_dd_bps(N, HW, C))) ? 1 : 0;
 }
 
 extern "C" int igan_bias_act_noise_fwd(igan_stream_t stream_, const float* x, const float* noise, const float* strength,
@@ -334,17 +482,11 @@
 extern "C" int igan_bias_act_noise_bwd(igan_stream_t stream_, const float* dy, const float* y, const float* noise,
                                        float* dx, float* db, float* dstrength, float* workspace,
                                        int rows, int C, int act, float alpha, float gain) {
-    using namespace igan;
-    IGAN_REQUIRE(dy && y && dx && workspace, "bias_act_noise_bwd: null buffer");
-    IGAN_REQUIRE((noise == nullptr) || (dstrength != nullptr), "bias_act_noise_bwd: noise given without dstrength");
-    if (int rc = ban_check("bias_act_noise_bwd", rows, C, act, gain)) return rc;
-    IGAN_REQUIRE((((uintptr_t)dy | (uintptr_t)y | (uintptr_t)dx) & 15) == 0, "bias_act_noise_bwd: buffers must be 16-byte aligned");
-    BanArgs a{dy, y, noise, nullptr, nullptr, dx, workspace, rows, C, act, alpha, gain};
-    const int blocks = ban_blocks(rows, C);
-    dim3 grid(blocks, ceil_div(C / 4, 256));
-    hipLaunchKernelGGL(ban_bwd_kernel, grid, dim3(256), 0, (hipStream_t)stream_, a);
-    hipLaunchKernelGGL(ban_final_kernel, dim3(ceil_div(C + 1, 16)), dim3(256), 0, (hipStream_t)stream_,
-                       (const float*)workspace, db, noise ? dstrength : nullptr, blocks, C);
-    IGAN_LAUNCH_CHECK("bias_act_noise_bwd launch");
-    return IGAN_OK;
-}
+    return ban_bwd_impl(stream_, dy, y, noise, dx, db, dstrength, workspace, rows, C, act, alpha, gain, false, nullptr, 0, nullptr, nullptr);
+}
+
+extern "C" int igan_bias_act_noise_bwd_rows(igan_stream_t stream_, const float* dy, const float* y, const float* noise,
+                                            float* dx, float* db, float* dstrength, float* workspace,
+                                            int rows, int C, int act, float alpha, float gain, const float* dscale, int HW, void* rows_out, float* colmax) {
+    return ban_bwd_impl(stream_, dy, y, noise, dx, db, dstrength, workspace, rows, C, act, alpha, gain, true, dscale, HW, rows_out, colmax);
+}
diff --git a/inclusivegan_amd/csrc/conv2d_mfma.hip b/inclusivegan_amd/csrc/conv2d_mfma.hip
--- a/inclusivegan_amd/csrc/conv2d_mfma.hip
+++ b/inclusivegan_amd/csrc/conv2d_mfma.hip
@@ -1,4 +1,5 @@
 #include "igan_common.h"
+#include "row_image.h"
 #include <cmath>
 #include <cstdlib>
 #include <type_traits>
@@ -998,41 +999,12 @@
 
 
 typedef _Float16 f16x8 __attribute__((ext_vector_type(8)));
-constexpr int H_COLBLOCKS = 1024;
 constexpr int H_KSK = 2;
 __device__ unsigned long long g_f16_below_window = 0ull, g_f16_imaged = 0ull;
 __device__ unsigned long long g_f16_below_window_cols = 0ull, g_f16_imaged_cols = 0ull;
 
-__host__ __device__ inline size_t align256(size_t b) { return (b + 255) & ~(size_t)255; }
-inline size_t rows_part_bytes(size_t P_, size_t C) { return align256(4 * P_ * C + 4 * P_); }
 inline size_t cols_part_bytes(size_t P_, size_t C) { return align256(4 * P_ * C + 8 * C + 4 * (size_t)H_COLBLOCKS * C); }
 inline size_t filter_part_bytes(size_t taps, size_t Nn, size_t K) { return align256(4 * taps * Nn * K + 4 * Nn + 4 * taps * H_KSK * Nn); }
-
-__device__ __forceinline__ float scale_from_amax(float amax) {
-    int e = (int)((__float_as_uint(amax) >> 23) & 0xFFu);
-    e = max(15, min(e, 254));
-    return __uint_as_float((unsigned)(268 - e) << 23);
-}
-__device__ __forceinline__ float inv_scale_from_amax(float amax) {
-    int e = (int)((__float_as_uint(amax) >> 23) & 0xFFu);
-    e = max(15, min(e, 254));
-    return __uint_as_float((unsigned)(e - 14) << 23);
-}
-__device__ __forceinline__ void count_window(int below, unsigned long long* counter) {
-#ifdef IGAN_NO_WINDOW_COUNT
-    return;
-#endif
-#pragma unroll
-    for (int o = 32; o >= 1; o >>= 1) below += __shfl_xor(below, o);
-    if ((threadIdx.x & 63) == 0 && below != 0) atomicAdd(counter, (unsigned long long)below);
-}
-
-__device__ __forceinline__ void split2(float vs, unsigned short (&o)[2]) {
-    const _Float16 p0 = (_Float16)vs;
-    const _Float16 p1 = (_Float16)((vs - (float)p0) * 2048.0f);
-    o[0] = __builtin_bit_cast(unsigned short, p0);
-    o[1] = __builtin_bit_cast(unsigned short, p1);
-}
 
 __device__ __forceinline__ void load_unit16(const float* __restrict__ x, const float* __restrict__ scale, int p, int c, int C, int HW, float (&v)[16]) {
     const float4* src = reinterpret_cast<const float4*>(x + (size_t)p * C + 16 * c);
@@ -1090,9 +1062,9 @@
         for (int i = 0; i < 16; i++) {
             unsigned short o[2];
             const float vs = v[i] * S;
-            split2(vs, o);
+            split2_row(vs, o);
             pc[0][i] = o[0]; pc[1][i] = o[1];
-            below += (mine && vs != 0.0f && fabsf(vs) < 0x1p-12f) ? 1 : 0;
+            below += mine ? below_window(vs) : 0;
         }
         if (chunk != (int)blockIdx.x) __syncthreads();
         store_units(pc, stage, out, total, chunk);
@@ -1186,7 +1158,7 @@
         const float vs = v[i] * S[i];
         split2(vs, o);
         pc[0][i] = o[0]; pc[1][i] = o[1];
-        below += (mine && vs != 0.0f && fabsf(vs) < 0x1p-12f) ? 1 : 0;
+        below += mine ? below_window(vs) : 0;
     }
     count_window(below, &g_f16_below_window_cols);
 #ifndef IGAN_NO_WINDOW_COUNT
@@ -2739,7 +2711,7 @@
 }
 void launch_row_image(hipStream_t stream, const float* x, const float* scale, unsigned short* out, int P_, int HW, int C, float* colmax) {
     const int cpp = C / PK, total = P_ * cpp;
-    float* rowinv = reinterpret_cast<float*>(reinterpret_cast<unsigned char*>(out) + (size_t)P_ * C * 4);
+    float* rowinv = row_image_rowinv(out, (size_t)P_, (size_t)C);
     const int nchunks = igan::ceil_div(total, 256);
     const int grid = colmax ? std::min(nchunks, H_COLBLOCKS) : nchunks;
     hipLaunchKernelGGL(rows_f16_kernel, dim3(grid), dim3(256), 0, stream, x, scale, out, rowinv, colmax, total, cpp, ilog2(cpp), C, HW);
@@ -3010,6 +2982,11 @@
         const unsigned short* xp = reinterpret_cast<const unsigned short*>(p->x_pieces);
         unsigned short* wp = reinterpret_cast<unsigned short*>(p->workspace + partial_floats + planes_x_floats(p));
         const int cpp = p->Cin / PK;
+        if (planes_mode() == 2 && p->x_rows != nullptr) {
+            IGAN_REQUIRE(p->x_rows_bytes == igan_row_image_bytes(p->N, p->H * p->W, p->Cin) && (((uintptr_t)p->x_rows) & 15) == 0,
+                         "conv2d: x_rows is not a row image of this x (x_rows_bytes != igan_row_image_bytes(N, H*W, Cin), or not 16-byte aligned)");
+            xp = reinterpret_cast<const unsigned short*>(p->x_rows);
+        }
         if (xp == nullptr) {
             unsigned short* own = reinterpret_cast<unsigned short*>(p->workspace + partial_floats);
             if (a.diag_mode & 1) {}
@@ -3312,6 +3289,40 @@
 
 extern "C" int igan_conv_piece_form(void) { return planes_mode(); }
 
+int igan::f16_row_counters(unsigned long long** below, unsigned long long** imaged) {
+    static unsigned long long* cache[64][2] = {};
+    int dev = 0;
+    IGAN_HIP_CHECK(hipGetDevice(&dev), "f16_row_counters: hipGetDevice");
+    IGAN_REQUIRE(dev >= 0 && dev < 64, "f16_row_counters: device index out of range");
+    if (cache[dev][0] == nullptr) {
+        void *b = nullptr, *i = nullptr;
+        IGAN_HIP_CHECK(hipGetSymbolAddress(&b, HIP_SYMBOL(g_f16_below_window)), "f16_row_counters: hipGetSymbolAddress");
+        IGAN_HIP_CHECK(hipGetSymbolAddress(&i, HIP_SYMBOL(g_f16_imaged)), "f16_row_counters: hipGetSymbolAddress");
+        cache[dev][1] = reinterpret_cast<unsigned long long*>(i);
+        cache[dev][0] = reinterpret_cast<unsigned long long*>(b);
+    }
+    *below = cache[dev][0];
+    *imaged = cache[dev][1];
+    return IGAN_OK;
+}
+
+extern "C" size_t igan_row_image_bytes(int N, int HW, int C) {
+    if (planes_mode() != 2 || N < 1 || HW < 1 || C < PK || C % BK != 0 || !pow2(C / PK) || C / PK > 64) return 0;
+    if ((long long)N * HW * C * 6 >= 0x7FFFFF00LL) return 0;
+    return rows_part_bytes((size_t)N * HW, (size_t)C);
+}
+
+extern "C" int igan_row_image(igan_stream_t stream_, const float* x, const float* scale, void* out, int N, int HW, int C, float* colmax) {
+    using namespace igan;
+    IGAN_REQUIRE(x != nullptr && out != nullptr, "row_image: null buffer");
+    IGAN_REQUIRE(igan_row_image_bytes(N, HW, C) != 0, "row_image: igan_row_image_bytes() says this process / tensor takes none");
+    IGAN_REQUIRE((((uintptr_t)x | (uintptr_t)scale | (uintptr_t)out | (uintptr_t)colmax) & 15) == 0, "row_image: buffers must be 16-byte aligned");
+    IGAN_REQUIRE(colmax == nullptr || igan_colmax_floats(N, HW, C) != 0, "row_image: colmax given, but igan_colmax_floats() says this process / tensor takes none");
+    launch_row_image((hipStream_t)stream_, x, scale, reinterpret_cast<unsigned short*>(out), N * HW, HW, C, colmax);
+    IGAN_LAUNCH_CHECK("row_image launch");
+    return IGAN_OK;
+}
+
 extern "C" size_t igan_colmax_floats(int N, int HW, int C) {
     using namespace igan;
     if (planes_mode() != 2 || N < 1 || HW < 1 || C < 16 || C > 1024 || (C & (C - 1)) != 0) return 0;
diff --git a/inclusivegan_amd/csrc/igan_common.h b/inclusivegan_amd/csrc/igan_common.h
--- a/inclusivegan_amd/csrc/igan_common.h
+++ b/inclusivegan_amd/csrc/igan_common.h
@@ -46,6 +46,8 @@
 size_t thin_wgrad_workspace(const igan_conv2d_wgrad_params* p, int kind);
 void thin_wgrad(hipStream_t stream, const igan_conv2d_wgrad_params* p, int kind);
 
+int f16_row_counters(unsigned long long** below, unsigned long long** imaged);
+
 inline int ceil_div(int a, int b) { return (a + b - 1) / b; }
 inline long long ceil_div_ll(long long a, long long b) { return (a + b - 1) / b; }
 
diff --git a/inclusivegan_amd/csrc/row_image.h b/inclusivegan_amd/csrc/row_image.h
--- /dev/null
+++ b/inclusivegan_amd/csrc/row_image.h
@@ -0,0 +1,41 @@
+#pragma once
+#include <hip/hip_runtime.h>
+#include <cstddef>
+#include <cstdint>
+
+constexpr int H_COLBLOCKS = 1024;
+
+__host__ __device__ inline size_t align256(size_t b) { return (b + 255) & ~(size_t)255; }
+inline size_t rows_part_bytes(size_t P_, size_t C) { return align256(4 * P_ * C + 4 * P_); }
+inline float* row_image_rowinv(void* out, size_t P_, size_t C) { return reinterpret_cast<float*>(reinterpret_cast<unsigned char*>(out) + P_ * C * 4); }
+__host__ __device__ inline size_t row_image_index(size_t p, int c, int C, int q) { return (p * (size_t)(C >> 4) + (size_t)(c >> 4)) * 32 + (size_t)q * 16 + (size_t)(c & 15); }
+
+__device__ __forceinline__ float scale_from_amax(float amax) {
+    int e = (int)((__float_as_uint(amax) >> 23) & 0xFFu);
+    e = max(15, min(e, 254));
+    return __uint_as_float((unsigned)(268 - e) << 23);
+}
+__device__ __forceinline__ float inv_scale_from_amax(float amax) {
+    int e = (int)((__float_as_uint(amax) >> 23) & 0xFFu);
+    e = max(15, min(e, 254));
+    return __uint_as_float((unsigned)(e - 14) << 23);
+}
+__device__ __forceinline__ void split2(float vs, unsigned short (&o)[2]) {
+    const _Float16 p0 = (_Float16)vs;
+    const _Float16 p1 = (_Float16)((vs - (float)p0) * 2048.0f);
+    o[0] = __builtin_bit_cast(unsigned short, p0);
+    o[1] = __builtin_bit_cast(unsigned short, p1);
+}
+__device__ __forceinline__ void split2_row(float vs, unsigned short (&o)[2]) {
+    split2(vs, o);
+    if (vs == 0.0f) o[0] = o[1] = (unsigned short)(__float_as_uint(vs) >> 16);
+}
+__device__ __forceinline__ int below_window(float vs) { return (vs != 0.0f && fabsf(vs) < 0x1p-12f) ? 1 : 0; }
+__device__ __forceinline__ void count_window(int below, unsigned long long* counter) {
+#ifdef IGAN_NO_WINDOW_COUNT
+    return;
+#endif
+#pragma unroll
+    for (int o = 32; o >= 1; o >>= 1) below += __shfl_xor(below, o);
+    if ((threadIdx.x & 63) == 0 && below != 0) atomicAdd(counter, (unsigned long long)below);
+}
diff --git a/inclusivegan_amd/hip_ops.py b/inclusivegan_amd/hip_ops.py
--- a/inclusivegan_amd/hip_ops.py
+++ b/inclusivegan_amd/hip_ops.py
@@ -335,7 +335,7 @@
     return y
 
 
-def bias_act_noise_bwd_raw(dy, y, noise, act_idx, alpha, gain, want_db):
+def bias_act_noise_bwd_raw(dy, y, noise, act_idx, alpha, gain, want_db, rows_image=None, colmax=None):
     lib = _abi.get_plugin()
     _require_cuda_f32(dy, y, noise)
     rows, c = _rows_c(y)
@@ -344,6 +344,10 @@
     ws = torch.empty((int(lib.igan_bias_act_noise_workspace_floats(rows, c)),), device=y.device, dtype=torch.float32)
     db = torch.empty((c,), device=y.device, dtype=torch.float32) if want_db else None
     ds = torch.empty((), device=y.device, dtype=torch.float32) if noise is not None else None
+    if rows_image is not None:
+        _abi.check(lib.igan_bias_act_noise_bwd_rows(_stream(), _ptr(dy), _ptr(y), _ptr(noise), _ptr(dx), _ptr(db), _ptr(ds), _ptr(ws),
+                                                    rows, c, act_idx, float(alpha), float(gain), None, rows // y.shape[0], rows_image.data_ptr(), _ptr(colmax)))
+        return dx, db, ds
     _abi.check(lib.igan_bias_act_noise_bwd(_stream(), _ptr(dy), _ptr(y), _ptr(noise), _ptr(dx), _ptr(db), _ptr(ds), _ptr(ws),
                                            rows, c, act_idx, float(alpha), float(gain)))
     return dx, db, ds
@@ -532,6 +536,33 @@
     if fl == 0:
         return None
     return torch.empty((fl,), device=x.device, dtype=torch.float32)
+
+
+ROW_PRODUCER = os.environ.get('IGAN_ROW_PRODUCER', '1') != '0'
+_row_producer = {}
+
+
+def row_image_buffer(dxp, w, geom, in_hw, in_scale=None):
+    if not ROW_PRODUCER or _is_meta(dxp) or dxp.dim() != 4:
+        return None
+    n, c, h, wd = (int(v) for v in dxp.shape)
+    g = dgrad_geom(geom)
+    key = (n, c, h, wd, int(in_hw[0]), int(in_hw[1]), int(w.shape[2]), g, in_scale is not None)
+    nbytes = _row_producer.get(key)
+    if nbytes is None:
+        lib = _abi.get_plugin()
+        nbytes = 0
+        if lib.igan_bias_act_noise_image_ok(n, h * wd, c):
+            p = _abi.Conv2DParams(x=256, w=256, y=256, in_scale=(256 if in_scale is not None else None), N=n, H=h, W=wd, Cin=c, OH=int(in_hw[0]), OW=int(in_hw[1]),
+                                  Cout=int(w.shape[2]), KH=g.kh, KW=g.kw, stride=g.stride, up=g.up, pad_y=g.pad_y, pad_x=g.pad_x, w_transposed=1, splits=1, alpha=float(g.alpha))
+            buf = ctypes.create_string_buffer(128)
+            _abi.check(lib.igan_conv2d_kernel_name(ctypes.byref(p), buf, 128))
+            if buf.value.decode().startswith('conv_fwd_planes'):
+                nbytes = int(lib.igan_row_image_bytes(n, h * wd, c))
+        _row_producer[key] = nbytes
+    if nbytes == 0:
+        return None
+    return PieceImage(torch.empty(((nbytes + 3) // 4,), device=dxp.device, dtype=torch.float32), nbytes)
 
 
 _filter_bytes = {}
@@ -568,7 +599,7 @@
     return PieceImage(img, nbytes)
 
 
-def conv2d_raw(x, w, geom, out_hw, cout, w_transposed=False, in_scale=None, out_scale=None, bias=None, act=None, noise=None, strength=None, x_pieces=None, colmax=None):
+def conv2d_raw(x, w, geom, out_hw, cout, w_transposed=False, in_scale=None, out_scale=None, bias=None, act=None, noise=None, strength=None, x_pieces=None, colmax=None, x_rows=None):
     if _is_meta(x):
         return torch.empty((x.shape[0], cout, out_hw[0], out_hw[1]), device='meta')
     lib = _abi.get_plugin()
@@ -600,6 +631,9 @@
         p.x_pieces_bytes = x_pieces.nbytes
     if colmax is not None:
         p.x_colmax = colmax.data_ptr()
+    if x_rows is not None:
+        p.x_rows = x_rows.data_ptr()
+        p.x_rows_bytes = x_rows.nbytes
     wimg = _constant_filter_image(lib, w, geom, cin, cout, w_transposed)
     if wimg is not None:
         p.w_pieces = wimg.data_ptr()
@@ -813,12 +847,13 @@
             if need_w:
                 dw = ConvWgradFn.apply(x, dxp, ctx.geom)
             return dx, dw, db, None, None, None, None, None
-        dxp, db, _ = bias_act_noise_bwd_raw(dy, y, None, act_idx, alpha, gain, need_b)
         share = pieces_wanted(ctx.geom, x.shape[1], y.shape[1]) and need_x and need_w
+        dycm = colmax_buffer(y, share)
+        rimg = row_image_buffer(y, w, ctx.geom, ctx.in_hw) if need_x else None
+        dxp, db, _ = bias_act_noise_bwd_raw(dy, y, None, act_idx, alpha, gain, need_b, rows_image=rimg, colmax=(dycm if rimg is not None else None))
         dyp = to_pieces(dxp) if share else None
-        dycm = colmax_buffer(dxp, share)
         if need_x:
-            dx = conv2d_raw(dxp, w, dgrad_geom(ctx.geom), ctx.in_hw, w.shape[2], w_transposed=True, x_pieces=dyp, colmax=dycm)
+            dx = conv2d_raw(dxp, w, dgrad_geom(ctx.geom), ctx.in_hw, w.shape[2], w_transposed=True, x_pieces=dyp, colmax=dycm, x_rows=rimg)
         if need_w:
             dw = conv2d_wgrad_raw(x, dxp, ctx.geom, x_pieces=ctx.xp, dy_pieces=dyp, x_colmax=ctx.xcm, dy_colmax=dycm)
         return dx, dw, (db if need_b else None), None, None, None, None, None
@@ -981,7 +1016,7 @@
         return g_dy, g_x, g_w, g_s, g_d, None, None, None, None
 
 
-def bias_act_noise_bwd_dd_raw(dy, y, noise, strength, b, d, act_idx, alpha, gain):
+def bias_act_noise_bwd_dd_raw(dy, y, noise, strength, b, d, act_idx, alpha, gain, rows_image=None, colmax=None):
     lib = _abi.get_plugin()
     _require_cuda_f32(dy, y, noise, strength, b, d)
     y = nhwc(y)
@@ -993,6 +1028,10 @@
     ds = torch.empty((), device=y.device, dtype=torch.float32) if noise is not None else None
     dd = torch.empty((n, c), device=y.device, dtype=torch.float32)
     bcast = 1 if (noise is not None and noise.numel() == h * w and n > 1) else 0
+    if rows_image is not None:
+        _abi.check(lib.igan_bias_act_noise_bwd_dd_rows(_stream(), _ptr(dy), _ptr(y), _ptr(noise), _ptr(strength), _ptr(b), _ptr(d.contiguous()), _ptr(dx), _ptr(db),
+                                                       _ptr(ds), _ptr(dd), _ptr(ws), bcast, n, h * w, c, act_idx, float(alpha), float(gain), rows_image.data_ptr(), _ptr(colmax)))
+        return dx, db, ds, dd
     _abi.check(lib.igan_bias_act_noise_bwd_dd(_stream(), _ptr(dy), _ptr(y), _ptr(noise), _ptr(strength), _ptr(b), _ptr(d.contiguous()), _ptr(dx), _ptr(db),
                                               _ptr(ds), _ptr(dd), _ptr(ws), bcast, n, h * w, c, act_idx, float(alpha), float(gain)))
     return dx, db, ds, dd
@@ -1021,14 +1060,15 @@
         geom = ctx.geom
         need_x, need_w, need_s, need_d, need_b = [_needed(ctx, i) for i in range(5)]
         need_st = noise is not None and _needed(ctx, 6)
-        dxp, db, dst, dd = bias_act_noise_bwd_dd_raw(dy, y, noise, strength, b, d, act_idx, alpha, gain)
         dx = dw = ds = None
         in_hw = (x.shape[2], x.shape[3])
         share = pieces_wanted(geom, x.shape[1], y.shape[1]) and (need_x or need_s) and need_w
+        dycm = colmax_buffer(y, share)
+        rimg = row_image_buffer(y, w, geom, in_hw, in_scale=d) if (need_x or need_s) else None
+        dxp, db, dst, dd = bias_act_noise_bwd_dd_raw(dy, y, noise, strength, b, d, act_idx, alpha, gain, rows_image=rimg, colmax=(dycm if rimg is not None else None))
         dyp = to_pieces(dxp, d) if share else None
-        dycm = colmax_buffer(dxp, share)
         if need_x or need_s:
-            dxs = conv2d_raw(dxp, w, dgrad_geom(geom), in_hw, w.shape[2], w_transposed=True, in_scale=d, x_pieces=dyp, colmax=dycm)
+            dxs = conv2d_raw(dxp, w, dgrad_geom(geom), in_hw, w.shape[2], w_transposed=True, in_scale=d, x_pieces=dyp, colmax=dycm, x_rows=rimg)
             ds, dx = scale_dot_raw(x, dxs, s, want_scaled=need_x)
             if not need_s:
                 ds = None
```

Result: no change. 355.1 (-0.1%).
